# ShijieZhou-UCLA/feature-3dgs

Hardware: AMD Instinct MI355X
Metric: rendered Mpix/s of rasterizer fwd+bwd (train-step ms in ms_per_step), 1M Gaussians @1080p, feat_dim=32 (higher is better)
Workload: dtype f32 (blend-backward sums: bf16 x 2-term products, f32 accumulate); 1 GPU; c3: 1000000 Gaussians, 1920x1080, SH degree 3, feat_dim=32, one view per GPU (SURVEY.md 8d recipe, seed 0), fresh upstream gradients per step; P=1000000, parallelism=single GPU

## Files before the change

### feature-3dgs_amd/csrc/api.hip

```cpp

#include <algorithm>
#include <atomic>
#include <cstdarg>
#include <cstdio>
#include <cstdlib>
#include <cstring>
#include <initializer_list>
#include <limits>
#include <mutex>
#include <string>
#include <vector>

#include "common.h"

using namespace f3dgs;

namespace {

thread_local std::string g_err;
thread_local f3dgs_stage_fn g_feature_ready_fn = nullptr;
thread_local void* g_feature_ready_ctx = nullptr;
thread_local f3dgs_rows_fn g_rows_ready_fn = nullptr;
thread_local void* g_rows_ready_ctx = nullptr;
thread_local int g_rows_ready_chunks = 1;
// ... 95 lines not shown
    do {                                                                                       \
        hipError_t e_ = (expr);                                                                \
        if (e_ != hipSuccess) return fail(F3DGS_ERR_HIP, "%s failed: %s", #expr, hipGetErrorString(e_)); \
    } while (0)

bool profiling() { return options().profile != 0; }

struct PendingSpan {
    const char* name;
    hipEvent_t a, b;
};
std::mutex g_prof_mu;
std::vector<PendingSpan> g_pending;
std::vector<hipEvent_t> g_event_pool;
std::vector<std::pair<const char*, std::pair<double, long>>> g_totals;

void resolve_pending_locked();
constexpr size_t MAX_PENDING_SPANS = 4096;

hipEvent_t take_event_locked() {
    if (!g_event_pool.empty()) {
        hipEvent_t e = g_event_pool.back();
        g_event_pool.pop_back();
        return e;
    }
    hipEvent_t e = nullptr;
    (void)hipEventCreate(&e);
    return e;
}

struct StageTimer {
    hipStream_t s;
    bool on;
    bool blend_only;
    hipEvent_t prev;
    explicit StageTimer(hipStream_t st, bool allowed = true) : s(st), on(allowed && profiling()), blend_only(options().profile == 2), prev(nullptr) {
        if (on && !blend_only) {
            {
                std::lock_guard<std::mutex> lk(g_prof_mu);
                prev = take_event_locked();
            }
            (void)hipEventRecord(prev, s);
        }
    }
    ~StageTimer() {
        if (prev) {
            std::lock_guard<std::mutex> lk(g_prof_mu);
            g_pending.push_back({nullptr, prev, nullptr});
        }
    }
    StageTimer(const StageTimer&) = delete;
    StageTimer& operator=(const StageTimer&) = delete;
    void mark(const char* name) {
        if (!on) return;
        if (blend_only) {
            const bool opens = strcmp(name, "tile_sort") == 0 || strcmp(name, "zero") == 0;
            const bool closes = strcmp(name, "render_fwd") == 0 || strcmp(name, "render_bwd") == 0;
            if (!opens && !closes) return;
            hipEvent_t ev;
            {
                std::lock_guard<std::mutex> lk(g_prof_mu);
                if (g_pending.size() >= MAX_PENDING_SPANS) resolve_pending_locked();
                ev = take_event_locked();
            }
            (void)hipEventRecord(ev, s);
            if (opens) { prev = ev; return; }
            std::lock_guard<std::mutex> lk(g_prof_mu);
            if (prev) g_pending.push_back({name, prev, ev});
            g_pending.push_back({nullptr, ev, nullptr});
            prev = nullptr;
            return;
        }
        hipEvent_t e;
        {
            std::lock_guard<std::mutex> lk(g_prof_mu);
            if (g_pending.size() >= MAX_PENDING_SPANS) resolve_pending_locked();
            e = take_event_locked();
        }
        (void)hipEventRecord(e, s);
        {
            std::lock_guard<std::mutex> lk(g_prof_mu);
            g_pending.push_back({name, prev, e});
        }
        prev = e;
    }
};

void resolve_pending() {
    std::lock_guard<std::mutex> lk(g_prof_mu);
    resolve_pending_locked();
}

void resolve_pending_locked() {
    for (auto& p : g_pending) {
        if (p.name) {
            (void)hipEventSynchronize(p.b);
            float ms = 0;
            (void)hipEventElapsedTime(&ms, p.a, p.b);
            bool found = false;
            for (auto& t : g_totals)
                if (strcmp(t.first, p.name) == 0) { t.second.first += ms; t.second.second++; found = true; break; }
            if (!found) g_totals.push_back({p.name, {ms, 1}});
        } else {
            (void)hipEventSynchronize(p.a);
        }
        g_event_pool.push_back(p.a);
    }
    g_pending.clear();
}

int check_debug(int debug, hipStream_t s, const char* stage) {
    if (!debug) return F3DGS_OK;
    hipError_t e = hipStreamSynchronize(s);
    if (e == hipSuccess) e = hipGetLastError();
    if (e != hipSuccess) return fail(F3DGS_ERR_HIP, "stage '%s' failed: %s", stage, hipGetErrorString(e));
    return F3DGS_OK;
}

void fill_view(ViewParams& vp, const float* view, const float* proj, const float* campos, const float* bg, float tanx,
               float tany, int W, int H, float mod) {
    vp.view = view; vp.proj = proj; vp.campos = campos; vp.bg = bg;
    vp.tanx = tanx; vp.tany = tany;
    vp.fx = W / (2.0f * tanx); vp.fy = H / (2.0f * tany);
    vp.W = W; vp.H = H;
    vp.gx = (W + TILE - 1) / TILE; vp.gy = (H + TILE - 1) / TILE;
    vp.band0 = 0; vp.band1 = vp.gy;
    vp.scale_modifier = mod;
    vp.max_axis_ratio = 0.f;
}

int tile_cull_enabled() { return options().tile_cull ? 1 : 0; }

struct OptionDesc {
    const char* name;
    const char* env;
    int Options::*field;
    int dflt;
};
const OptionDesc kOptions[] = {
    {"tile_cull", "F3DGS_TILE_CULL", &Options::tile_cull, 1},
    {"feature_mfma", "F3DGS_FEATURE_MFMA", &Options::feature_mfma, 1},
    {"profile", "F3DGS_PROFILE", &Options::profile, 0},
    {"bwd_half", "F3DGS_BWD_HALF", &Options::bwd_half, 1},
    {"bwd_pl", "F3DGS_BWD_PL", &Options::bwd_pl, -1},
    {"bwd_order", "F3DGS_BWD_ORDER", &Options::bwd_order, 1},
    {"bwd_m44", "F3DGS_BWD_M44", &Options::bwd_m44, 1},
    {"bwd_split16", "F3DGS_BWD_SPLIT16", &Options::bwd_split16, 1},
    {"bwd_bf16", "F3DGS_BWD_BF16", &Options::bwd_bf16, -1},
    {"bwd_bf16_max_ratio", "F3DGS_BWD_BF16_MAX_RATIO", &Options::bwd_bf16_max_ratio, 16},
    {"bwd_wide8", "F3DGS_BWD_WIDE8", &Options::bwd_wide8, 1},
    {"fwd_wide", "F3DGS_FWD_WIDE", &Options::fwd_wide, 1},
    {"fwd_solo", "F3DGS_FWD_SOLO", &Options::fwd_solo, 1},
    {"sort_onesweep", "F3DGS_SORT_ONESWEEP", &Options::sort_onesweep, 0},
    {"sync_free", "F3DGS_SYNC_FREE", &Options::sync_free, -1},
    {"instance_capacity", "F3DGS_INSTANCE_CAPACITY", &Options::instance_capacity, 0},
    {"knn_outward", "F3DGS_KNN_OUTWARD", &Options::knn_outward, 1},
#ifdef F3DGS_DEV
    {"dev", "F3DGS_DEV_BITS", &Options::dev, 0},
#endif
};

bool misaligned16(std::initializer_list<const void*> ptrs) {
    uintptr_t bits = 0;
    for (const void* p : ptrs) bits |= reinterpret_cast<uintptr_t>(p);
    return (bits & 15) != 0;
}

int tile_bits(int tiles) {
    int b = 0;
    while ((1 << b) < tiles) b++;
    return b < 1 ? 1 : b;
}

}

namespace f3dgs {
Options& options() {
    static Options o = [] {
        Options v{};
        for (const OptionDesc& d : kOptions) {
            const char* e = getenv(d.env);
            v.*(d.field) = e ? atoi(e) : d.dflt;
        }
        return v;
    }();
    return o;
}
}

namespace {
struct CountReadback {
    uint32_t* host = nullptr;
    uint32_t* dev = nullptr;
    hipEvent_t done = nullptr;
    int device = -1;
    hipStream_t stream = nullptr;
    bool in_graph = false;
};
struct CountHint { bool known = false; uint32_t own = 0, ref = 0; };
thread_local CountHint g_count_hint[64];
thread_local const uint32_t* g_last_forward_words = nullptr;
bool stream_is_capturing(hipStream_t s) {
    hipStreamCaptureStatus st = hipStreamCaptureStatusNone;
    if (hipStreamIsCapturing(s, &st) != hipSuccess) { (void)hipGetLastError(); return false; }
    return st == hipStreamCaptureStatusActive;
}
const hipStream_t kSpareSlot = reinterpret_cast<hipStream_t>(~uintptr_t(0));
bool make_count_slot(std::vector<CountReadback>& slots, int dev, hipStream_t s) {
    CountReadback rb;
    void* p = nullptr;
    if (hipHostMalloc(&p, 64, hipHostMallocPortable | hipHostMallocMapped) != hipSuccess) { (void)hipGetLastError(); return false; }
    rb.host = static_cast<uint32_t*>(p);
    void* d = nullptr;
    if (hipHostGetDevicePointer(&d, p, 0) != hipSuccess || hipEventCreateWithFlags(&rb.done, hipEventDisableTiming) != hipSuccess) {
        (void)hipGetLastError();
        (void)hipHostFree(p);
        return false;
    }
    rb.dev = static_cast<uint32_t*>(d);
    rb.device = dev;
    rb.stream = s;
    memset(p, 0, 64);
    if (slots.size() >= 64) {
        for (size_t i = 0; i < slots.size(); i++)
            if (!slots[i].in_graph && slots[i].stream != kSpareSlot) {
                (void)hipEventDestroy(slots[i].done);
                (void)hipHostFree(slots[i].host);
                slots.erase(slots.begin() + (long)i);
                break;
            }
    }
    slots.push_back(rb);
    return true;
}
CountReadback* count_readback(hipStream_t s, bool may_create) {
    thread_local std::vector<CountReadback> slots;
    int dev = 0;
    if (hipGetDevice(&dev) != hipSuccess) return nullptr;
    auto find = [&](hipStream_t key) -> CountReadback* {
        for (CountReadback& rb : slots)
            if (rb.device == dev && rb.stream == key) return &rb;
        return nullptr;
    };
    if (!may_create) {
        if (CountReadback* rb = find(s)) return rb;
        if (CountReadback* spare = find(kSpareSlot)) { spare->stream = s; return spare; }
        return nullptr;
    }
    if (!find(kSpareSlot)) (void)make_count_slot(slots, dev, kSpareSlot);
    if (!find(s) && !make_count_slot(slots, dev, s)) return nullptr;
    return find(s);
}
}

extern "C" {

int f3dgs_version(void) { return 32200; }

int f3dgs_last_backward_contraction(void) { return g_last_bwd_bf16.load(); }

const uint32_t* f3dgs_forward_counts(void) { return g_last_forward_words; }

int f3dgs_set_option(const char* name, int value) {
    if (!name) return fail(F3DGS_ERR_INVALID_ARGUMENT, "null option name");
    for (const OptionDesc& d : kOptions)
        if (strcmp(d.name, name) == 0) {
            options().*(d.field) = value;
            return F3DGS_OK;
        }
    return fail(F3DGS_ERR_INVALID_ARGUMENT, "unknown option '%s'", name);
}

int f3dgs_get_option(const char* name, int* value) {
    if (!name || !value) return fail(F3DGS_ERR_INVALID_ARGUMENT, "null argument");
    for (const OptionDesc& d : kOptions)
        if (strcmp(d.name, name) == 0) {
            *value = options().*(d.field);
            return F3DGS_OK;
        }
    return fail(F3DGS_ERR_INVALID_ARGUMENT, "unknown option '%s'", name);
}

const char* f3dgs_option_name(int index) {
    const int n = (int)(sizeof(kOptions) / sizeof(kOptions[0]));
    return (index >= 0 && index < n) ? kOptions[index].name : nullptr;
}

const char* f3dgs_last_error(void) { return g_err.c_str(); }

void f3dgs_set_feature_grad_ready_callback(f3dgs_stage_fn fn, void* ctx) {
    g_feature_ready_fn = fn;
    g_feature_ready_ctx = ctx;
}

void f3dgs_set_feature_grad_accumulate(int on) { g_feature_accumulate = on ? 1 : 0; }

int f3dgs_set_feature_grad_lowres(const float* gx, int Hg, int Wg, const float* scale) {
    if (!gx) { g_lowres = LowresGrad(); return F3DGS_OK; }
    if (Hg <= 0 || Wg <= 0) return fail(F3DGS_ERR_INVALID_ARGUMENT, "bad low-resolution size %d x %d", Hg, Wg);
    g_lowres.gx = gx; g_lowres.scale = scale; g_lowres.Hg = Hg; g_lowres.Wg = Wg;
    return F3DGS_OK;
}

int f3dgs_debug_band_order(int gx, int gy, int tile_row_begin, int tile_row_end, uint32_t* tiles_out) {
    if (gx <= 0 || gy <= 0 || !tiles_out) return fail(F3DGS_ERR_INVALID_ARGUMENT, "bad grid");
    int b0r, b1r;
    clamp_band(tile_row_begin, tile_row_end, gy, &b0r, &b1r);
    uint32_t b0 = 0, tb = 0;
    band_perm_params(gx, gy, b0r, b1r, &b0, &tb);
    const uint32_t T = (uint32_t)gx * (uint32_t)gy;
    for (uint32_t v = 0; v < T; v++) tiles_out[v] = band_perm(v, T, b0, tb);
    return tb != 0 ? 1 : 0;
}

void f3dgs_set_tile_band(int tile_row_begin, int tile_row_end) {
    g_band_begin = tile_row_begin;
    g_band_end = tile_row_end;
}

void f3dgs_set_grad_rows_ready_callback(f3dgs_rows_fn fn, void* ctx, int chunks) {
    g_rows_ready_fn = fn;
    g_rows_ready_ctx = ctx;
    g_rows_ready_chunks = chunks > 0 ? chunks : 1;
}

int f3dgs_mark_visible(int P, const float* means3D, const float* viewmatrix, const float* projmatrix,
                       uint8_t* present, void* stream) {
    hipStream_t s = static_cast<hipStream_t>(stream);
    if (P < 0) return fail(F3DGS_ERR_INVALID_ARGUMENT, "P < 0");
    if (P == 0) return F3DGS_OK;
    if (!means3D || !viewmatrix || !present) return fail(F3DGS_ERR_INVALID_ARGUMENT, "null pointer");
    (void)projmatrix;
    launch_mark_visible(P, means3D, viewmatrix, present, s);
    HIP_TRY(hipGetLastError());
    return F3DGS_OK;
}

int f3dgs_forward(f3dgs_resize_fn geometry_resize, void* geometry_ctx, f3dgs_resize_fn binning_resize,
                  void* binning_ctx, f3dgs_resize_fn image_resize, void* image_ctx, int P, int D, int M, int C,
                  const float* background, int width, int height, const float* means3D, const float* shs,
                  const float* colors_precomp, const float* semantic_feature, const float* opacities,
                  const float* scales, float scale_modifier, const float* rotations, const float* cov3D_precomp,
                  const float* viewmatrix, const float* projmatrix, const float* cam_pos, float tan_fovx,
                  float tan_fovy, int prefiltered, float* out_color, float* out_feature_map, float* out_depth,
                  int* radii, int debug, void* stream, int* num_rendered) {
    hipStream_t s = static_cast<hipStream_t>(stream);
    (void)prefiltered;
    if (num_rendered) *num_rendered = 0;
    if (P < 0 || C < 0 || width <= 0 || height <= 0) return fail(F3DGS_ERR_INVALID_ARGUMENT, "bad sizes");
    if (!geometry_resize || !binning_resize || !image_resize) return fail(F3DGS_ERR_INVALID_ARGUMENT, "null resize hook");
    if (!out_color || !out_depth || (C > 0 && !out_feature_map)) return fail(F3DGS_ERR_INVALID_ARGUMENT, "null output");
    const size_t HW = (size_t)width * height;
    if (P == 0) {
        const bool cap0 = stream_is_capturing(s);
        HIP_TRY(zero_fill(out_color, 3 * HW * sizeof(float), cap0, s));
        HIP_TRY(zero_fill(out_depth, HW * sizeof(float), cap0, s));
        if (C) HIP_TRY(zero_fill(out_feature_map, (size_t)C * HW * sizeof(float), cap0, s));
        return F3DGS_OK;
    }
    if (!means3D || !opacities || !viewmatrix || !projmatrix || !background)
        return fail(F3DGS_ERR_INVALID_ARGUMENT, "null input");
    if (!colors_precomp && !shs) return fail(F3DGS_ERR_INVALID_ARGUMENT, "need shs or colors_precomp");
    if (!colors_precomp && !cam_pos) return fail(F3DGS_ERR_INVALID_ARGUMENT, "SH colours need cam_pos");
    if (!cov3D_precomp && (!scales || !rotations))
        return fail(F3DGS_ERR_INVALID_ARGUMENT, "need scales+rotations or cov3D_precomp");
    if (C > 0 && !semantic_feature) return fail(F3DGS_ERR_INVALID_ARGUMENT, "semantic_feature is null but C > 0");
    if (shs && (D < 0 || D > 3 || (D + 1) * (D + 1) > M))
        return fail(F3DGS_ERR_INVALID_ARGUMENT, "SH degree %d needs %d coefficients, M = %d", D, (D + 1) * (D + 1), M);
    if (misaligned16({shs, rotations, semantic_feature}))
        return fail(F3DGS_ERR_INVALID_ARGUMENT, "shs, rotations and semantic_feature must be 16-byte aligned (f3dgs.h, Alignment)");

    int rc = F3DGS_OK;
    ViewParams vp;
    fill_view(vp, viewmatrix, projmatrix, cam_pos, background, tan_fovx, tan_fovy, width, height, scale_modifier);
    vp.max_axis_ratio = 1.001f * (float)options().bwd_bf16_max_ratio;
    if (g_band_begin != 0 || g_band_end != 0) clamp_band(g_band_begin, g_band_end, vp.gy, &vp.band0, &vp.band1);
    const int2 band = make_int2(vp.band0, vp.band1);
    const size_t tiles = (size_t)vp.gx * vp.gy;

    size_t geom_bytes = 0, img_bytes = 0, bin_bytes = 0;
    GeomState::carve(nullptr, P, &geom_bytes);
    char* geom_ptr = geometry_resize(geometry_ctx, geom_bytes);
    if (!geom_ptr) return fail(F3DGS_ERR_ALLOC, "geometry buffer allocation of %zu bytes failed", geom_bytes);
    GeomState geom = GeomState::carve(geom_ptr, P, nullptr);
    ImageState::carve(nullptr, HW, tiles, &img_bytes);
    char* img_ptr = image_resize(image_ctx, img_bytes);
    if (!img_ptr) return fail(F3DGS_ERR_ALLOC, "image buffer allocation of %zu bytes failed", img_bytes);
    ImageState img = ImageState::carve(img_ptr, HW, tiles, nullptr);
    const bool onesweep = options().sort_onesweep != 0 && tiles <= 65536;

    const bool capturing = stream_is_capturing(s);
    const int sf_opt = options().sync_free;
    const bool sync_free = !onesweep && (sf_opt > 0 || (sf_opt < 0 && capturing));
    if (capturing && !sync_free)
        return fail(F3DGS_ERR_UNSUPPORTED, "the stream is being captured into a graph: the forward call reads the instance count on the host "
                    "unless option sync_free is 1 or -1 (and sort_onesweep = 0)");
    if (capturing && debug) return fail(F3DGS_ERR_UNSUPPORTED, "debug = 1 synchronises after every stage: not inside a graph capture");
    int dev_index = 0;
    HIP_TRY(hipGetDevice(&dev_index));
    if (dev_index < 0 || dev_index >= 64) return fail(F3DGS_ERR_UNSUPPORTED, "device index %d", dev_index);
    CountHint& hint = g_count_hint[dev_index];

    StageTimer tm(s, !capturing);
    const int cull = tile_cull_enabled();
    launch_preprocess(P, D, M, means3D, scales, rotations, opacities, shs, cov3D_precomp, colors_precomp, vp, radii,
                      geom, cull, s);
    if ((rc = check_debug(debug, s, "preprocess"))) return rc;
    tm.mark("preprocess");
    if (onesweep) launch_sort_prologue(geom, (size_t)P, s);
    CountReadback* rbp = count_readback(s, !capturing);
    if (!rbp)
        return capturing ? fail(F3DGS_ERR_UNSUPPORTED, "graph capture: run one forward call on this stream (same host thread) before capturing - "
                                "the pinned count words are allocated on a stream's first call")
                         : fail(F3DGS_ERR_ALLOC, "pinned read-back buffer / event creation failed");
    CountReadback& rb = *rbp;
    if (capturing) rb.in_graph = true;
    g_last_forward_words = rb.host;
    if (onesweep) {
        HIP_TRY(hipMemcpyAsync(rb.host, geom.counters, 8, hipMemcpyDeviceToHost, s));
        HIP_TRY(hipEventRecord(rb.done, s));
    }

    const TotalsJob tj = {geom.ref_partial, (P + 255) / 256, geom.counters, rb.dev, capturing ? nullptr : rb.done};
    const OffsetSumsJob sums = {geom.tiles_touched, geom.scan_tmp, geom.scan_sub};
    bool sums_done = false;
    bool counts_in_a = false;
    if (onesweep) launch_depth_sort_onesweep(geom, (size_t)P, s);
    else HIP_TRY(launch_depth_sort(geom.depth_key, geom.key_a, geom.val_a, geom.key_b, geom.val_b, (size_t)P, geom.hist, &tj, s, &sums, &sums_done, &counts_in_a));
    if ((rc = check_debug(debug, s, "depth sort"))) return rc;
    tm.mark("depth_sort");
    const uint32_t* order = geom.val_a;
    const uint32_t* counts_in_order = counts_in_a ? geom.key_a : nullptr;

    if (!onesweep && !sums_done) {
        if (counts_in_order) launch_offset_sums(counts_in_order, nullptr, (size_t)P, geom.scan_tmp, geom.scan_sub, s);
        else launch_offset_sums(geom.tiles_touched, order, (size_t)P, geom.scan_tmp, geom.scan_sub, s);
    }

    bool known = false;
    uint32_t N = 0, n_ref = 0, cap = 0;
    auto read_counts = [&]() -> int {
        HIP_TRY(hipEventSynchronize(rb.done));
        N = rb.host[0]; n_ref = rb.host[1];
        note_frame(geom_ptr, (onesweep || rb.host[2] != 0u) ? 1.f : 0.f, vp.band0, vp.band1);
        hint.known = true; hint.own = N; hint.ref = n_ref;
        known = true;
        if (N >= (1u << 30) || n_ref >= (1u << 31)) return fail(F3DGS_ERR_UNSUPPORTED, "more than 2^30 instances");
        return F3DGS_OK;
    };
    if (sync_free && (options().instance_capacity > 0 || hint.known)) {
        unsigned long long want = options().instance_capacity > 0 ? (unsigned long long)options().instance_capacity
                                                                  : (unsigned long long)hint.own + hint.own / 4 + 4096ull;
        if (options().instance_capacity <= 0 && hint.own <= (uint32_t)SMALL_SORT_MAX && want > (unsigned long long)SMALL_SORT_MAX)
            want = SMALL_SORT_MAX;
        cap = (uint32_t)std::min(want, (1ull << 30) - 1ull);
    } else if (capturing) {
        return fail(F3DGS_ERR_UNSUPPORTED, "graph capture: no provision for the instance lists - run one forward call on this thread and device "
                    "before capturing, or set option instance_capacity");
    } else {
        if ((rc = read_counts())) return rc;
        cap = N;
    }
    tm.mark("scan+sync");

    const int bits = tile_bits((int)tiles);
    const int passes = (bits + RADIX_BITS - 1) / RADIX_BITS;
    BinState bin;
    for (;;) {
        const uint32_t n_carve = known ? N : cap;
        BinState::carve(nullptr, n_carve, &bin_bytes, tiles);
        char* bin_ptr = binning_resize(binning_ctx, bin_bytes);
        if (!bin_ptr) return fail(F3DGS_ERR_ALLOC, "binning buffer allocation of %zu bytes failed", bin_bytes);
        bin = BinState::carve(bin_ptr, n_carve, nullptr, tiles);
        rb.host[3] = n_carve;
        uint32_t* in_tile = (passes % 2 == 0) ? bin.tile_sorted : bin.tile_tmp;
        uint32_t* in_id = (passes % 2 == 0) ? bin.point_list : bin.id_tmp;
        if (onesweep) {
            HIP_TRY(hipMemsetAsync(img.tile_len, 0, tiles * sizeof(uint32_t), s));
            launch_emit_scan(P, geom, bin, order, vp.gx, vp.gy, band, cull, in_tile, in_id, N, bin.ranges_enc, s);
            if ((rc = check_debug(debug, s, "emit"))) return rc;
            tm.mark("emit");
            launch_tile_sort_onesweep(geom, bin, N, passes, bin.ranges_enc, s);
            if ((rc = check_debug(debug, s, "tile sort"))) return rc;
            tm.mark("tile_sort");
        } else if (known && N == 0) {
            HIP_TRY(hipMemsetAsync(bin.ranges_enc, 0xFF, tiles * sizeof(uint2), s));
            HIP_TRY(hipMemsetAsync(img.tile_len, 0, tiles * sizeof(uint32_t), s));
        } else {
            launch_emit_instances(P, geom, order, counts_in_order, vp.gx, vp.gy, band, cull, in_tile, in_id, bin.ranges_enc, img.tile_len, n_carve,
                                  known ? nullptr : geom.counters, capturing ? rb.dev + 4 : nullptr, s);
            if ((rc = check_debug(debug, s, "emit"))) return rc;
            tm.mark("emit");
            launch_radix_sort_pairs(bin.tile_sorted, bin.point_list, bin.tile_tmp, bin.id_tmp, n_carve, bits, bin.hist, true,
                                    bin.ranges_enc, s, known ? nullptr : geom.counters);
            if ((rc = check_debug(debug, s, "tile sort"))) return rc;
            tm.mark("tile_sort");
        }

        launch_render_forward(vp, C, bin.ranges_enc, img.ranges, bin.point_list, geom.rec, semantic_feature, img.final_T,
                              img.n_contrib, out_color, out_feature_map, out_depth, img.tile_len, s);
        if ((rc = check_debug(debug, s, "render"))) return rc;
        tm.mark("render_fwd");
        if (known || capturing) break;
        if ((rc = read_counts())) return rc;
        if (N <= cap) break;
    }
    if (capturing) {
        note_frame(geom_ptr, 2.f, vp.band0, vp.band1);
        n_ref = std::max(1u, hint.ref);
    }
    if (num_rendered) *num_rendered = (int)n_ref;
    HIP_TRY(hipGetLastError());
    return F3DGS_OK;
}

size_t f3dgs_backward_scratch_bytes(int P, int C) {
    (void)C;
    return ((size_t)(P > 0 ? P : 0) * GREC * sizeof(float) + ALIGN - 1) & ~(ALIGN - 1);
}

int f3dgs_backward(int P, int D, int M, int C, int R, const float* background, int width, int height,
                   const float* means3D, const float* shs, const float* colors_precomp,
                   const float* semantic_feature, const float* scales, float scale_modifier, const float* rotations,
                   const float* cov3D_precomp, const float* viewmatrix, const float* projmatrix, const float* campos,
                   float tan_fovx, float tan_fovy, const int* radii, const char* geom_buffer,
                   const char* binning_buffer, const char* image_buffer, const float* dL_dpix,
                   const float* dL_dfeaturepix, const float* dL_depths, float* dL_dmean2D, float* dL_dconic,
                   float* dL_dopacity, float* dL_dcolor, float* dL_dsemantic_feature, float* dL_dmean3D,
                   float* dL_dcov3D, float* dL_dsh, float* dL_dscale, float* dL_drot, float* dL_dz, void* scratch,
                   int debug, void* stream) {
    hipStream_t s = static_cast<hipStream_t>(stream);
    (void)semantic_feature;
    (void)colors_precomp;
    const LowresGrad lowres = g_lowres;
    g_lowres = LowresGrad();
    if (P < 0 || C < 0 || R < 0) return fail(F3DGS_ERR_INVALID_ARGUMENT, "bad sizes");
    if (P == 0) return F3DGS_OK;
    if (!geom_buffer || !image_buffer || (R > 0 && !binning_buffer))
        return fail(F3DGS_ERR_INVALID_ARGUMENT, "null state buffer");
    if (!radii) return fail(F3DGS_ERR_INVALID_ARGUMENT, "radii is required");
    if (lowres.gx) {
        if (C == 0) return fail(F3DGS_ERR_INVALID_ARGUMENT, "a low-resolution feature-map gradient was set but C = 0");
        if (lowres.Hg > height || lowres.Wg > width)
            return fail(F3DGS_ERR_UNSUPPORTED, "low-resolution feature-map gradient %d x %d is larger than the image %d x %d: "
                        "apply the transposed resize outside (f3dgs_feature_l1 with d_feature_map)", lowres.Hg, lowres.Wg, height, width);
        if (!options().feature_mfma)
            return fail(F3DGS_ERR_UNSUPPORTED, "the low-resolution feature-map gradient is taken by the pixel-lane backward (option feature_mfma = 1)");
    }
    if (!dL_dpix || !dL_depths || (C > 0 && !dL_dfeaturepix && !lowres.gx)) return fail(F3DGS_ERR_INVALID_ARGUMENT, "null upstream grad");
    if (!dL_dmean2D || !dL_dopacity || !dL_dcolor || !dL_dmean3D || !dL_dcov3D || (C > 0 && !dL_dsemantic_feature))
        return fail(F3DGS_ERR_INVALID_ARGUMENT, "null output");
    if (M > 0 && shs && !dL_dsh) return fail(F3DGS_ERR_INVALID_ARGUMENT, "dL_dsh is null");
    if (shs && dL_dsh && (D < 0 || D > 3 || (D + 1) * (D + 1) > M))
        return fail(F3DGS_ERR_INVALID_ARGUMENT, "SH degree %d needs %d coefficients, M = %d", D, (D + 1) * (D + 1), M);
    if (scales && (!dL_dscale || !dL_drot || !rotations)) return fail(F3DGS_ERR_INVALID_ARGUMENT, "scale/rot grads null");
    if (!scratch) return fail(F3DGS_ERR_INVALID_ARGUMENT, "scratch is null");
    if (misaligned16({shs, rotations, dL_dsh, dL_drot, dL_dconic, dL_dsemantic_feature, scratch}))
        return fail(F3DGS_ERR_INVALID_ARGUMENT, "shs, rotations, dL_dsh, dL_drot, dL_dconic, dL_dsemantic_feature and scratch must be "
                    "16-byte aligned (f3dgs.h, Alignment)");

    int rc = F3DGS_OK;
    ViewParams vp;
    fill_view(vp, viewmatrix, projmatrix, campos, background, tan_fovx, tan_fovy, width, height, scale_modifier);
    const size_t HW = (size_t)width * height, tiles = (size_t)vp.gx * vp.gy;
    GeomState geom = GeomState::carve(const_cast<char*>(geom_buffer), P, nullptr);
    const uint32_t* point_list = BinState::list_of(binning_buffer);
    ImageState img = ImageState::carve(const_cast<char*>(image_buffer), HW, tiles, nullptr);
    float* grec = static_cast<float*>(scratch);

    const bool capturing = stream_is_capturing(s);
    if (capturing && debug) return fail(F3DGS_ERR_UNSUPPORTED, "debug = 1 synchronises after every stage: not inside a graph capture");
    StageTimer tm(s, !capturing);
    HIP_TRY(zero_fill(grec, (size_t)P * GREC * sizeof(float), capturing, s));
    if (C > 0 && !g_feature_accumulate) HIP_TRY(zero_fill(dL_dsemantic_feature, (size_t)P * C * sizeof(float), capturing, s));
    tm.mark("zero");
    int contraction = options().bwd_bf16 > 0 ? 1 : 0;
    {
        float long_axis = 1.f;
        const bool noted = frame_note(geom_buffer, vp.gy, &long_axis, &vp.band0, &vp.band1);
        if (options().bwd_bf16 < 0) {
            contraction = (noted && long_axis == 0.f) ? 1 : 2;
// ... 461 lines not shown
```

### feature-3dgs_amd/csrc/binding.cpp

```cpp

#include <ATen/hip/impl/HIPGuardImplMasqueradingAsCUDA.h>
#include <ATen/hip/impl/HIPStreamMasqueradingAsCUDA.h>
#include <torch/extension.h>

#include <array>
#include <exception>
#include <stdexcept>
#include <string>
#include <tuple>
#include <vector>

#include "../../include/f3dgs.h"

namespace py = pybind11;

namespace {

const float* fptr(const torch::Tensor& t) { return t.numel() ? t.data_ptr<float>() : nullptr; }

char* resize_hook(void* ctx, size_t n) {
    auto* t = static_cast<torch::Tensor*>(ctx);
    t->resize_({(long long)n});
    return reinterpret_cast<char*>(t->data_ptr());
}
// ... 1072 lines not shown
                "densify_gather: override_row must be int32 of the same length");
    TORCH_CHECK(srcs.size() == dsts.size() && srcs.size() == modes.size() && srcs.size() == overrides.size(), "densify_gather: list lengths differ");
    std::vector<f3dgs_densify_tensor> table(srcs.size());
    for (size_t i = 0; i < srcs.size(); i++) {
        const auto& a = srcs[i];
        auto& d = dsts[i];
        TORCH_CHECK(a.is_cuda() && d.is_cuda() && a.scalar_type() == torch::kFloat32 && d.scalar_type() == torch::kFloat32, "densify_gather: float32 HIP tensors only");
        TORCH_CHECK(a.is_contiguous() && d.is_contiguous(), "densify_gather: contiguous tensors only");
        int64_t width = 1;
        for (int64_t k = 1; k < a.dim(); k++) width *= a.size(k);
        TORCH_CHECK(a.dim() >= 1 && width >= 1, "densify_gather: tensors are (rows, ...) with non-empty rows");
        TORCH_CHECK((size_t)d.numel() >= n_out * (size_t)width, "densify_gather: destination ", i, " too small");
        table[i].src = a.data_ptr<float>();
        table[i].dst = d.data_ptr<float>();
        table[i].width = (int)width;
        table[i].mode = (int)modes[i];
        table[i].override_src = nullptr;
        if (modes[i] == F3DGS_DENSIFY_OVERRIDE_CHILD) {
            const auto& o = overrides[i];
            TORCH_CHECK(o.is_cuda() && o.scalar_type() == torch::kFloat32 && o.is_contiguous(), "densify_gather: override must be a contiguous float32 HIP tensor");
            table[i].override_src = o.numel() ? o.data_ptr<float>() : a.data_ptr<float>();
        }
    }
    c10::hip::HIPGuardMasqueradingAsCUDA guard(src_row.device());
    check_status(f3dgs_densify_gather(n_out, src_row.data_ptr<int32_t>(), kind.data_ptr<uint8_t>(), override_row.data_ptr<int32_t>(),
                                      (int)table.size(), table.data(), current_stream(src_row)),
                 "densify_gather");
}

}

PYBIND11_MODULE(_C, m) {
    m.def("rasterize_gaussians", &RasterizeGaussians);
    m.def("rasterize_gaussians_backward", &RasterizeGaussiansBackward);
    m.def("mark_visible", &markVisible);
    m.def("feature_l1", &FeatureL1, py::arg("feature_map"), py::arg("gt"), py::arg("weight"), py::arg("bias"), py::arg("dense") = true);
    m.def("set_feature_grad_lowres", [](py::object gx, py::object scale) {
              auto& h = feature_grad_lowres();
              h.first = gx.is_none() ? torch::Tensor() : gx.cast<torch::Tensor>();
              h.second = (gx.is_none() || scale.is_none()) ? torch::Tensor() : scale.cast<torch::Tensor>();
          },
          py::arg("gx"), py::arg("scale") = py::none(),
          "gx (Hg, Wg, C) float32 = dL/d(resized feature map) as feature_l1 returns it, scale = 0-dim device tensor or None: the NEXT "
          "rasterize_gaussians_backward call takes its feature-map gradient from there (transposed resize applied per tile); None clears");
    m.def("feature_decode", &FeatureDecode);
    m.def("image_loss_forward", &ImageLossForward, py::arg("image"), py::arg("gt"), py::arg("lambda_dssim"), py::arg("want_grad"),
          py::arg("per_image") = false);
    m.def("image_loss_backward", &ImageLossBackward, py::arg("image"), py::arg("gt"), py::arg("scratch"), py::arg("upstream"),
          py::arg("lambda_dssim"), py::arg("mode"));
    m.attr("IMAGE_LOSS_L1_DSSIM") = (int)F3DGS_IMAGE_LOSS_L1_DSSIM;
    m.attr("IMAGE_LOSS_SSIM") = (int)F3DGS_IMAGE_LOSS_SSIM;
    m.attr("IMAGE_LOSS_SSIM_PER_IMAGE") = (int)F3DGS_IMAGE_LOSS_SSIM_PER_IMAGE;
    m.def("image_metrics", &ImageMetrics, py::arg("image"), py::arg("gt"), py::arg("image_format"), py::arg("gt_format"), py::arg("flags"),
          py::arg("want_ssim") = true);
    m.attr("IMAGE_F32") = (int)F3DGS_IMAGE_F32;
    m.attr("IMAGE_U8_PLANAR") = (int)F3DGS_IMAGE_U8_PLANAR;
    m.attr("IMAGE_U8_INTERLEAVED") = (int)F3DGS_IMAGE_U8_INTERLEAVED;
    m.attr("METRICS_QUANTIZE_IMAGE") = (int)F3DGS_METRICS_QUANTIZE_IMAGE;
    m.attr("METRICS_QUANTIZE_GT") = (int)F3DGS_METRICS_QUANTIZE_GT;
    m.def("edit_select", &EditSelect, py::arg("features"), py::arg("text"), py::arg("positive_mask"), py::arg("first_positive"),
          py::arg("variant"), py::arg("threshold") = py::none(), py::arg("normalize_inplace") = false, py::arg("want_score") = false,
          py::arg("opacity") = py::none());
    m.def("segment", &Segment, py::arg("feature_map"), py::arg("text"), py::arg("Hs"), py::arg("Ws"), py::arg("weight"), py::arg("bias"),
          py::arg("flags"), py::arg("want_score"));
    m.def("contributions", &Contributions, py::arg("geomBuffer"), py::arg("binningBuffer"), py::arg("imgBuffer"), py::arg("P"),
          py::arg("num_rendered"), py::arg("H"), py::arg("W"), py::arg("masks") = py::none(), py::arg("acc") = py::none(),
          py::arg("wmax") = py::none(), py::arg("want_pixel") = true);
    m.attr("CONTRIB_MAX_MASKS") = (int)F3DGS_CONTRIB_MAX_MASKS;
    m.def("label_votes", &LabelVotes, py::arg("geomBuffer"), py::arg("binningBuffer"), py::arg("imgBuffer"), py::arg("P"),
          py::arg("num_rendered"), py::arg("H"), py::arg("W"), py::arg("labels"), py::arg("L"), py::arg("acc"));
    m.attr("LABEL_VOTES_MAX_LABELS") = (int)F3DGS_LABEL_VOTES_MAX_LABELS;
    m.def("instance_associate", &InstanceAssociate, py::arg("acc_view"), py::arg("acc"), py::arg("count"), py::arg("dropped"),
          py::arg("iou_thresh"), py::arg("min_weight"));
    m.def("instance_merge", &InstanceMerge, py::arg("acc_view"), py::arg("mapping"), py::arg("acc"), py::arg("clear_view"));
    m.attr("INSTANCE_MAX_MASKS") = (int)F3DGS_INSTANCE_MAX_MASKS;
    m.attr("INSTANCE_MAX_INSTANCES") = (int)F3DGS_INSTANCE_MAX_INSTANCES;
    m.def("feature_pca_moments", &FeaturePcaMoments, py::arg("feature_map"), py::arg("stride"));
    m.def("feature_pca_project", &FeaturePcaProject, py::arg("feature_map"), py::arg("mean"), py::arg("components"),
          py::arg("lo") = py::none(), py::arg("hi") = py::none());
    m.attr("FEATURE_PCA_MAX_CHANNELS") = (int)F3DGS_FEATURE_PCA_MAX_CHANNELS;
    m.def("view_normals", &ViewNormals, py::arg("depth"), py::arg("projection_matrix"), py::arg("inv_full_proj"), py::arg("chw") = false,
          py::arg("half") = false);
    m.def("view_gradient", &ViewGradient, py::arg("image"));
    m.def("view_curvature", &ViewCurvature, py::arg("depth"), py::arg("projection_matrix"), py::arg("inv_full_proj"));
    m.def("view_minmax", &ViewMinmax, py::arg("field"));
    m.def("view_palette", &ViewPalette, py::arg("field"), py::arg("minmax"), py::arg("lut"), py::arg("mode"), py::arg("want_float") = true,
          py::arg("want_u8") = false);
    m.def("view_bytes", &ViewBytes, py::arg("image"));
    m.attr("VIEW_TILE") = (int)F3DGS_VIEW_TILE;
    m.attr("VIEW_PALETTE_MINMAX") = (int)F3DGS_VIEW_PALETTE_MINMAX;
    m.attr("VIEW_PALETTE_MAX") = (int)F3DGS_VIEW_PALETTE_MAX;
    m.attr("VIEW_PALETTE_MAX_ENTRIES") = (int)F3DGS_VIEW_PALETTE_MAX_ENTRIES;
    m.attr("SEGMENT_ROUND_HALF") = (int)F3DGS_SEGMENT_ROUND_HALF;
    m.attr("SEGMENT_TEXT_NORMALIZED") = (int)F3DGS_SEGMENT_TEXT_NORMALIZED;
    m.attr("SEGMENT_MAX_TEXTS") = (int)F3DGS_SEGMENT_MAX_TEXTS;
    m.def("seg_metrics", &SegMetrics, py::arg("teacher"), py::arg("student"), py::arg("gt"), py::arg("num_labels"), py::arg("num_classes"),
          py::arg("carry_counts"), py::arg("carry_scalars"), py::arg("want_scores"));
    m.def("seg_colorize", &SegColorize, py::arg("labels"), py::arg("palette"), py::arg("image"), py::arg("mode"), py::arg("a"), py::arg("b"),
          py::arg("fill"));
    m.def("sam_masks", &SamMasks, py::arg("low_res"), py::arg("iou_preds"), py::arg("pred_iou_thresh"), py::arg("S"), py::arg("ih"),
          py::arg("iw"), py::arg("H"), py::arg("W"), py::arg("FH"), py::arg("FW"), py::arg("cx0"), py::arg("cy0"), py::arg("t"), py::arg("t_hi"),
          py::arg("t_lo"), py::arg("stability_thresh"), py::arg("edge_filter"));
    m.def("sam_upscale", &SamUpscale, py::arg("low_res"), py::arg("S"), py::arg("ih"), py::arg("iw"), py::arg("H"), py::arg("W"), py::arg("t"),
          py::arg("out_bool"));
    m.def("box_nms", &BoxNms, py::arg("boxes"), py::arg("categories"), py::arg("iou_threshold"), py::arg("order"));
    m.def("mask_rle_count", &MaskRleCount, py::arg("packed"), py::arg("index"), py::arg("FH"));
    m.def("mask_rle_emit", &MaskRleEmit, py::arg("packed"), py::arg("index"), py::arg("FH"), py::arg("lens"), py::arg("ends"), py::arg("out"),
          py::arg("head"));
    m.def("mask_unpack", &MaskUnpack, py::arg("packed"), py::arg("index"), py::arg("FH"));
    m.def("mask_instance_map", &MaskInstanceMap, py::arg("packed"), py::arg("index"), py::arg("FH"));
    m.def("mask_regions", &MaskRegions, py::arg("packed"), py::arg("index"), py::arg("FH"), py::arg("area_thresh"), py::arg("holes"),
          py::arg("run_capacity"));
    m.attr("BOX_NMS_MAX") = (int)F3DGS_BOX_NMS_MAX;
    m.attr("LABELS_U8") = (int)F3DGS_LABELS_U8;
    m.attr("LABELS_I32") = (int)F3DGS_LABELS_I32;
    m.attr("LABELS_I64") = (int)F3DGS_LABELS_I64;
    m.attr("SEG_COLOR_MASK") = (int)F3DGS_SEG_COLOR_MASK;
    m.attr("SEG_COLOR_BLEND") = (int)F3DGS_SEG_COLOR_BLEND;
    m.attr("SEG_COLOR_STRIP") = (int)F3DGS_SEG_COLOR_STRIP;
    m.attr("EDIT_SELECT") = (int)F3DGS_EDIT_SELECT;
    m.attr("EDIT_DELETE") = (int)F3DGS_EDIT_DELETE;
    m.attr("EDIT_TEXT_NORMALIZED") = (int)F3DGS_EDIT_TEXT_NORMALIZED;
    m.attr("EDIT_FILL_UNSELECTED") = (int)F3DGS_EDIT_FILL_UNSELECTED;
    m.attr("EDIT_MAX_TEXTS") = (int)F3DGS_EDIT_MAX_TEXTS;
    m.attr("EDIT_MAX_TEXT_ELEMENTS") = (int)F3DGS_EDIT_MAX_TEXT_ELEMENTS;
    m.def("adam_step", &AdamStep, py::arg("param"), py::arg("grad"), py::arg("exp_avg"), py::arg("exp_avg_sq"), py::arg("lr"),
          py::arg("beta1"), py::arg("beta2"), py::arg("eps"), py::arg("step"), py::arg("row_mask") = py::none());
    m.def("adam_step_multi", &AdamStepMulti, py::arg("params"), py::arg("grads"), py::arg("exp_avgs"), py::arg("exp_avg_sqs"), py::arg("lrs"),
          py::arg("beta1"), py::arg("beta2"), py::arg("eps"), py::arg("steps"), py::arg("row_mask") = py::none());
    m.def("densify_gather", &DensifyGather);
    m.def("version", []() { return f3dgs_version(); });
    m.def("set_feature_grad_hook", [](py::object fn) { feature_grad_hook() = std::move(fn); },
          "callable(dL_dsemantic_feature) run inside rasterize_gaussians_backward once that tensor is final on the stream; None removes it");
    m.def("set_feature_grad_accumulator", [](py::object t) {
              if (t.is_none()) feature_grad_accumulator() = torch::Tensor();
              else feature_grad_accumulator() = t.cast<torch::Tensor>();
          },
          "tensor (P*C float32, contiguous, on the op's device) that the following backward calls ADD dL/dsemantic_feature into "
          "(they then return an empty tensor for that gradient); None restores the default");
    m.def("set_grad_rows_hook", [](py::object fn, int chunks) { grad_rows_hook() = std::move(fn); grad_rows_chunks() = chunks > 0 ? chunks : 1; },
          py::arg("fn"), py::arg("chunks") = 4,
          "callable(row_begin, row_end, grads: dict) run inside rasterize_gaussians_backward after each of `chunks` row ranges of the "
          "per-Gaussian gradients is final on the stream; None removes it");
    m.def("set_option", [](const std::string& name, int value) { check_status(f3dgs_set_option(name.c_str(), value), "set_option"); });
    m.def("set_tile_band", [](int row_begin, int row_end) { f3dgs_set_tile_band(row_begin, row_end); }, py::arg("tile_row_begin"), py::arg("tile_row_end"),
          "forward calls of this thread list and blend only tile rows [begin, end) of the view (0, 0: the whole view); include/f3dgs.h");
    m.def("forward_counts", []() -> py::object {
        const uint32_t* w = f3dgs_forward_counts();
        if (!w) return py::none();
        const volatile uint32_t* v = w;
        return py::make_tuple((long long)v[0], (long long)v[1], (long long)v[2], (long long)v[3], (long long)v[4]);
    }, "(entries of the instance lists, the reference's num_rendered, long-axis flag, entries provided for, sticky no-room word) of the "
       "calling thread's most recent forward call - final once that frame's work has completed; None before the first call");
    m.def("forward_counts_address", []() { return (uintptr_t)f3dgs_forward_counts(); },
          "host address of the five uint32 words of forward_counts() (0 before the first call): a captured step keeps it and reads the words after a replay");
    m.def("clear_forward_overflow", [](uintptr_t address) { if (address) reinterpret_cast<volatile uint32_t*>(address)[4] = 0u; },
          "clears the sticky no-room word behind an address returned by forward_counts_address()");
    m.def("last_backward_contraction", []() { return f3dgs_last_backward_contraction(); },
          "1: the last blend backward of this process contracted on bf16 matrix instructions (two-term operands); 0: exact fp32; -1: none yet");
    m.def("get_option", [](const std::string& name) {
        int v = 0;
        check_status(f3dgs_get_option(name.c_str(), &v), "get_option");
        return v;
    });
    m.def("profile_reset", []() { f3dgs_profile_reset(); });
    m.def("profile_read", []() {
        const char* names[64];
        double ms[64];
        long calls[64];
        const int n = f3dgs_profile_read(names, ms, calls, 64);
        std::vector<std::tuple<std::string, double, long>> out;
        for (int i = 0; i < n; i++) out.emplace_back(names[i], ms[i], calls[i]);
        return out;
    });
}
```

### feature-3dgs_amd/csrc/binning.hip

```cpp

#include <atomic>
#include "common.h"
#include "lookback.h"

namespace f3dgs {

namespace {

__global__ void __launch_bounds__(256) scan_reduce_kernel(const uint32_t* __restrict__ in,
                                                          const uint32_t* __restrict__ gather, size_t n,
                                                          uint32_t* __restrict__ block_sums, uint32_t* __restrict__ sub) {
    __shared__ uint32_t sh[8];
    const size_t base = (size_t)blockIdx.x * SCAN_CHUNK;
    const int lane = threadIdx.x & 63, w = threadIdx.x >> 6;
    uint32_t v[16];
#pragma unroll
    for (int k = 0; k < 16; k++) {
        const size_t i = base + (size_t)k * 256 + threadIdx.x;
        v[k] = i < n ? (gather ? in[gather[i]] : in[i]) : 0u;
    }
    uint32_t acc = 0;
#pragma unroll
    for (int k = 0; k < 16; k++) {
        uint32_t r = v[k];
#pragma unroll
        for (int d = 32; d >= 1; d >>= 1) r += (uint32_t)__shfl_xor((int)r, d, 64);
        if (lane == 0) sub[(size_t)blockIdx.x * 64 + 4 * k + w] = r;
        acc += v[k];
    }
    uint32_t tot;
    block_excl_scan_256(acc, sh, &tot);
    if (threadIdx.x == 0) block_sums[blockIdx.x] = tot;
}


template <int THREADS>
__device__ __forceinline__ void run_totals_job(const TotalsJob& tj) {
    __shared__ uint32_t shc[3][THREADS / 64];
    uint32_t v = 0, u = 0, ar = 0;
    for (int i = threadIdx.x; i < tj.n_partial; i += THREADS) {
        v += tj.partial[i]; u += tj.partial[tj.n_partial + i]; ar = max(ar, tj.partial[2 * tj.n_partial + i]);
    }
#pragma unroll
    for (int d = 32; d >= 1; d >>= 1) {
        v += (uint32_t)__shfl_xor((int)v, d, 64);
        u += (uint32_t)__shfl_xor((int)u, d, 64);
        ar = max(ar, (uint32_t)__shfl_xor((int)ar, d, 64));
    }
    if ((threadIdx.x & 63) == 0) { shc[0][threadIdx.x >> 6] = v; shc[1][threadIdx.x >> 6] = u; shc[2][threadIdx.x >> 6] = ar; }
    __syncthreads();
    if (threadIdx.x == 0) {
        uint32_t ref = 0, own = 0, arm = 0;
        for (int k = 0; k < THREADS / 64; k++) { ref += shc[0][k]; own += shc[1][k]; arm = max(arm, shc[2][k]); }
        tj.counters[0] = own; tj.counters[1] = ref; tj.counters[2] = arm; tj.counters[3] = 0u;
        if (tj.host) {
            __hip_atomic_store(&tj.host[0], own, __ATOMIC_RELAXED, __HIP_MEMORY_SCOPE_SYSTEM);
            __hip_atomic_store(&tj.host[1], ref, __ATOMIC_RELAXED, __HIP_MEMORY_SCOPE_SYSTEM);
            __hip_atomic_store(&tj.host[2], arm, __ATOMIC_RELAXED, __HIP_MEMORY_SCOPE_SYSTEM);
            __threadfence_system();
        }
    }
}

template <int BITS, int ITEMS>
__global__ void __launch_bounds__(SORT_THREADS) radix_hist_kernel(const uint32_t* __restrict__ keys, size_t n,
                                                                  int shift, uint32_t nb,
                                                                  uint32_t* __restrict__ hist, TotalsJob tj,
                                                                  const uint32_t* __restrict__ n_dev) {
    constexpr int BINS = 1 << BITS;
    constexpr int CHUNK = SORT_THREADS * ITEMS;
    __shared__ uint32_t h[BINS];
    if (n_dev) { const size_t nd = *n_dev; n = nd <= n ? nd : 0; }
    const size_t base = (size_t)blockIdx.x * CHUNK;
    uint32_t key[ITEMS];
#pragma unroll
    for (int k = 0; k < ITEMS; k++) {
        const size_t i = base + (size_t)k * SORT_THREADS + threadIdx.x;
        key[k] = i < n ? keys[i] : 0u;
    }
    if (tj.partial && blockIdx.x == 0) run_totals_job<SORT_THREADS>(tj);
    for (int d = threadIdx.x; d < BINS; d += SORT_THREADS) h[d] = 0;
    __syncthreads();
#pragma unroll
    for (int k = 0; k < ITEMS; k++) {
        const size_t i = base + (size_t)k * SORT_THREADS + threadIdx.x;
        if (i < n) atomicAdd(&h[(key[k] >> shift) & (BINS - 1)], 1u);
    }
    __syncthreads();
    for (int d = threadIdx.x; d < BINS; d += SORT_THREADS) hist[(size_t)d * nb + blockIdx.x] = h[d];
}

constexpr int ROWSCAN_GROUPS = 8;
__global__ void __launch_bounds__(256) radix_rowscan_kernel(uint32_t* __restrict__ hist, uint32_t nb,
                                                            uint32_t* __restrict__ totals) {
    __shared__ uint32_t sh[8];
    __shared__ uint4 wtot[ROWSCAN_GROUPS];
    uint32_t* row = hist + (size_t)blockIdx.x * nb;
    const int lane = threadIdx.x & 63, w = threadIdx.x >> 6;
    uint32_t v[ROWSCAN_GROUPS], inc[ROWSCAN_GROUPS];
#pragma unroll
    for (int k = 0; k < ROWSCAN_GROUPS; k++) {
        const uint32_t i = (uint32_t)k * 256 + threadIdx.x;
        const uint32_t r = row[i < nb ? i : 0u];
        v[k] = i < nb ? r : 0u;
    }
#pragma unroll
    for (int k = 0; k < ROWSCAN_GROUPS; k++) {
        inc[k] = (uint32_t)k * 256 < nb ? wave_incl_scan(v[k], lane) : 0u;
        if (lane == 63) (&wtot[k].x)[w] = inc[k];
    }
    __syncthreads();
    uint32_t carry = 0;
#pragma unroll
    for (int k = 0; k < ROWSCAN_GROUPS; k++) {
        const uint4 t = wtot[k];
        const uint32_t before = carry + (w > 0 ? t.x : 0u) + (w > 1 ? t.y : 0u) + (w > 2 ? t.z : 0u);
        const uint32_t i = (uint32_t)k * 256 + threadIdx.x;
        if (i < nb) row[i] = before + inc[k] - v[k];
        carry += t.x + t.y + t.z + t.w;
    }
    for (uint32_t base = ROWSCAN_GROUPS * 256; base < nb; base += 256) {
        const uint32_t i = base + threadIdx.x;
        const uint32_t v = i < nb ? row[i] : 0;
        uint32_t tot;
        const uint32_t ex = block_excl_scan_256(v, sh, &tot);
        if (i < nb) row[i] = carry + ex;
        carry += tot;
    }
    if (threadIdx.x == 0) totals[blockIdx.x] = carry;
}

__device__ __forceinline__ void record_range(uint2* ranges_enc, uint32_t tile, bool first, bool last, uint32_t pos) {
    if (first) atomicMin(&ranges_enc[tile].x, pos);
    if (last) atomicMin(&ranges_enc[tile].y, 0xFFFFFFFFu - (pos + 1u));
}

template <int BITS, int ITEMS, bool REORDER, bool RANGES, bool COUNTS = false>
__global__ void __launch_bounds__(SORT_THREADS)
radix_scatter_kernel(const uint32_t* __restrict__ keys_in, const uint32_t* __restrict__ vals_in,
                     uint32_t* __restrict__ keys_out, uint32_t* __restrict__ vals_out, size_t n, int shift,
                     uint32_t nb, const uint32_t* __restrict__ hist, const uint32_t* __restrict__ totals,
                     uint2* __restrict__ ranges_enc, const uint32_t* __restrict__ n_dev,
                     const uint32_t* __restrict__ payload) {
    constexpr int BINS = 1 << BITS;
    constexpr int CHUNK = SORT_THREADS * ITEMS;
    constexpr int BPT = BINS >= SORT_THREADS ? BINS / SORT_THREADS : 1;
    static_assert(BINS >= SORT_THREADS ? BINS % SORT_THREADS == 0 : true, "whole bins per thread");
    if (n_dev) {
        const size_t nd = *n_dev;
        n = nd <= n ? nd : 0;
        if ((size_t)blockIdx.x * CHUNK >= n) return;
    }
    __shared__ uint32_t cnt[4][BINS];
    __shared__ uint32_t sh[8];
    __shared__ uint32_t gbase[REORDER ? BINS : 1];
    __shared__ uint32_t lstart[REORDER ? BINS : 1];
    __shared__ uint32_t skey[REORDER ? CHUNK : 1];
    __shared__ uint32_t sval[REORDER ? CHUNK : 1];
    volatile uint32_t* vcnt = &cnt[0][0];
    const int lane = threadIdx.x & 63, w = threadIdx.x >> 6;
    for (int d = threadIdx.x; d < 4 * BINS; d += SORT_THREADS) (&cnt[0][0])[d] = 0;
    __syncthreads();

    const size_t wbase = (size_t)blockIdx.x * CHUNK + (size_t)w * (ITEMS * 64);
    uint32_t key[ITEMS];
    constexpr bool VAL_FIRST = REORDER || COUNTS;
    uint32_t val[VAL_FIRST ? ITEMS : 1];
    uint32_t rank[ITEMS];
    const unsigned long long lt_mask = (1ull << lane) - 1ull;
#pragma unroll
    for (int k = 0; k < ITEMS; k++) {
        const size_t i = wbase + (size_t)k * 64 + lane;
        key[k] = i < n ? keys_in[i] : 0xFFFFFFFFu;
        if constexpr (VAL_FIRST) val[k] = (vals_in && i < n) ? vals_in[i] : (uint32_t)i;
    }
#pragma unroll
    for (int k = 0; k < ITEMS; k++) {
        const size_t i = wbase + (size_t)k * 64 + lane;
        const bool valid = i < n;
        const uint32_t d = (key[k] >> shift) & (BINS - 1);
        const unsigned long long vm = __ballot(valid);
        uint32_t p_lo = (uint32_t)vm, p_hi = (uint32_t)(vm >> 32);
#pragma unroll
        for (int b = 0; b < BITS; b++) {
            const uint32_t x = 0u - ((d >> b) & 1u);
            const unsigned long long nm = ~__ballot(x != 0u);
            p_lo &= (uint32_t)nm ^ x;
            p_hi &= (uint32_t)(nm >> 32) ^ x;
        }
        const unsigned long long peers = ((unsigned long long)p_hi << 32) | p_lo;
        const uint32_t before = __popcll(peers & lt_mask);
        const uint32_t old = vcnt[w * BINS + d];
        if (valid && before == 0) vcnt[w * BINS + d] = old + (uint32_t)__popcll(peers);
        rank[k] = old + before;
    }
    uint32_t pay[(COUNTS && !REORDER) ? ITEMS : 1];
    (void)pay;
    if constexpr (COUNTS && !REORDER) {
#pragma unroll
        for (int k = 0; k < ITEMS; k++) {
            const size_t i = wbase + (size_t)k * 64 + lane;
            pay[k] = payload[i < n ? val[k] : 0u];
        }
    }
    __syncthreads();
    {
        uint32_t tot[BPT], run = 0, blk[BPT], brun = 0;
#pragma unroll
        for (int q = 0; q < BPT; q++) {
            const uint32_t d = threadIdx.x * BPT + q;
            const bool own = BINS >= SORT_THREADS || d < (uint32_t)BINS;
            tot[q] = own ? totals[d] : 0u;
            run += tot[q];
            blk[q] = own ? cnt[0][d] + cnt[1][d] + cnt[2][d] + cnt[3][d] : 0u;
            brun += blk[q];
        }
        uint32_t digit_base = block_excl_scan_256(run, sh, nullptr);
        uint32_t local_base = REORDER ? block_excl_scan_256(brun, sh, nullptr) : 0;
#pragma unroll
        for (int q = 0; q < BPT; q++) {
            const uint32_t d = threadIdx.x * BPT + q;
            if (BINS < SORT_THREADS && d >= (uint32_t)BINS) break;
            const uint32_t g = digit_base + hist[(size_t)d * nb + blockIdx.x];
            if (REORDER) { gbase[d] = g; lstart[d] = local_base; }
            uint32_t r2 = REORDER ? local_base : g;
#pragma unroll
            for (int k = 0; k < 4; k++) {
                const uint32_t c = cnt[k][d];
                cnt[k][d] = r2;
                r2 += c;
            }
            digit_base += tot[q];
            local_base += blk[q];
        }
    }
    __syncthreads();
    if (REORDER) {
#pragma unroll
        for (int k = 0; k < ITEMS; k++) {
            const size_t i = wbase + (size_t)k * 64 + lane;
            if (i < n) {
                const uint32_t d = (key[k] >> shift) & (BINS - 1);
                const uint32_t lp = cnt[w][d] + rank[k];
                skey[lp] = key[k];
                if constexpr (REORDER) sval[lp] = val[k];
            }
        }
        __syncthreads();
        const size_t cbase = (size_t)blockIdx.x * CHUNK;
        const uint32_t have = (uint32_t)min((size_t)CHUNK, n - cbase);
        if constexpr (COUNTS) {
            static_assert(!RANGES, "the depth sort records no ranges");
            uint32_t pos[ITEMS], id[ITEMS], c[ITEMS];
#pragma unroll
            for (int k = 0; k < ITEMS; k++) {
                const uint32_t j = (uint32_t)k * SORT_THREADS + threadIdx.x;
                const uint32_t jj = j < have ? j : 0u;
                const uint32_t d = (skey[jj] >> shift) & (BINS - 1);
                pos[k] = gbase[d] + (jj - lstart[d]);
                id[k] = sval[jj];
                c[k] = payload[id[k]];
            }
#pragma unroll
            for (int k = 0; k < ITEMS; k++) {
                const uint32_t j = (uint32_t)k * SORT_THREADS + threadIdx.x;
                if (j < have) {
                    keys_out[pos[k]] = c[k];
                    vals_out[pos[k]] = id[k];
                }
            }
        } else {
#pragma unroll
            for (int k = 0; k < ITEMS; k++) {
                const uint32_t j = (uint32_t)k * SORT_THREADS + threadIdx.x;
                if (j < have) {
                    const uint32_t kk = skey[j];
                    const uint32_t d = (kk >> shift) & (BINS - 1);
                    const uint32_t pos = gbase[d] + (j - lstart[d]);
                    keys_out[pos] = kk;
                    vals_out[pos] = sval[j];
                    if (RANGES) record_range(ranges_enc, kk, j == 0 || skey[j - 1] != kk, j + 1 == have || skey[j + 1] != kk, pos);
                }
            }
        }
    } else {
#pragma unroll
        for (int k = 0; k < ITEMS; k++) {
            const size_t i = wbase + (size_t)k * 64 + lane;
            if (i < n) {
                const uint32_t d = (key[k] >> shift) & (BINS - 1);
                const uint32_t pos = cnt[w][d] + rank[k];
                if constexpr (COUNTS) {
                    keys_out[pos] = pay[k];
                    vals_out[pos] = val[k];
                } else {
                    keys_out[pos] = key[k];
                    vals_out[pos] = vals_in ? vals_in[i] : (uint32_t)i;
                }
            }
        }
    }
}


template <int ITEMS, bool WRITE_KEYS, bool RANGES>
__global__ void __launch_bounds__(SORT_THREADS)
onesweep_pass_kernel(const uint32_t* __restrict__ keys_in, const uint32_t* __restrict__ vals_in,
                     uint32_t* __restrict__ keys_out, uint32_t* __restrict__ vals_out, size_t n, int shift,
                     const uint32_t* __restrict__ digit_totals, uint32_t* __restrict__ status,
                     uint32_t* __restrict__ ticket, uint2* __restrict__ ranges) {
    constexpr int BINS = 256;
    constexpr int CHUNK = SORT_THREADS * ITEMS;
    __shared__ uint32_t cnt[4][BINS];
    __shared__ uint32_t sh[8];
    __shared__ uint32_t gbase[BINS];
    __shared__ uint32_t lstart[BINS];
    __shared__ uint32_t skey[CHUNK];
    __shared__ uint32_t sval[CHUNK];
    __shared__ uint32_t s_vb;
    volatile uint32_t* vcnt = &cnt[0][0];
    const int lane = threadIdx.x & 63, w = threadIdx.x >> 6;
    if (threadIdx.x == 0) s_vb = atomicAdd(ticket, 1u);
    for (int d = threadIdx.x; d < 4 * BINS; d += SORT_THREADS) (&cnt[0][0])[d] = 0;
    __syncthreads();
    const uint32_t vb = s_vb;

    const size_t cbase = (size_t)vb * CHUNK;
    const size_t wbase = cbase + (size_t)w * (ITEMS * 64);
    uint32_t key[ITEMS];
    uint32_t rank[ITEMS];
    const unsigned long long lt_mask = (1ull << lane) - 1ull;
#pragma unroll
    for (int k = 0; k < ITEMS; k++) {
        const size_t i = wbase + (size_t)k * 64 + lane;
        const bool valid = i < n;
        key[k] = valid ? keys_in[i] : 0xFFFFFFFFu;
        const uint32_t d = (key[k] >> shift) & (BINS - 1);
        unsigned long long peers = __ballot(valid);
#pragma unroll
        for (int b = 0; b < 8; b++) {
            const bool bit = (d >> b) & 1;
            const unsigned long long m = __ballot(bit);
            peers &= bit ? m : ~m;
        }
        const uint32_t before = __popcll(peers & lt_mask);
        const uint32_t old = vcnt[w * BINS + d];
        if (valid && before == 0) vcnt[w * BINS + d] = old + (uint32_t)__popcll(peers);
        rank[k] = old + before;
    }
    __syncthreads();
    {
        const uint32_t d = threadIdx.x;
        const uint32_t blk = cnt[0][d] + cnt[1][d] + cnt[2][d] + cnt[3][d];
        const uint32_t total = digit_totals[d];
        const uint32_t digit_base = block_excl_scan_256(total, sh, nullptr);
        const uint32_t local_base = block_excl_scan_256(blk, sh, nullptr);
        const uint32_t before_me = lookback(status + d, BINS, vb, blk);
        gbase[d] = digit_base + before_me;
        lstart[d] = local_base;
        uint32_t r2 = local_base;
#pragma unroll
        for (int k = 0; k < 4; k++) {
            const uint32_t c = cnt[k][d];
            cnt[k][d] = r2;
            r2 += c;
        }
    }
    __syncthreads();
#pragma unroll
    for (int k = 0; k < ITEMS; k++) {
        const size_t i = wbase + (size_t)k * 64 + lane;
        if (i < n) {
            const uint32_t d = (key[k] >> shift) & (BINS - 1);
            const uint32_t lp = cnt[w][d] + rank[k];
            skey[lp] = key[k];
            sval[lp] = vals_in ? vals_in[i] : (uint32_t)i;
        }
    }
    __syncthreads();
    const uint32_t have = (uint32_t)min((size_t)CHUNK, n - cbase);
#pragma unroll
    for (int k = 0; k < ITEMS; k++) {
        const uint32_t j = (uint32_t)k * SORT_THREADS + threadIdx.x;
        if (j < have) {
            const uint32_t kk = skey[j];
            const uint32_t d = (kk >> shift) & (BINS - 1);
            const uint32_t pos = gbase[d] + (j - lstart[d]);
            if (WRITE_KEYS) keys_out[pos] = kk;
            vals_out[pos] = sval[j];
            if (RANGES) record_range(ranges, kk, j == 0 || skey[j - 1] != kk, j + 1 == have || skey[j + 1] != kk, pos);
        }
    }
}

__global__ void __launch_bounds__(256)
sort_prologue_kernel(const uint32_t* __restrict__ keys, size_t n, uint32_t* __restrict__ depth_hist,
                     const uint32_t* __restrict__ partial, int n_partial, uint32_t* __restrict__ counters,
                     uint32_t* __restrict__ zero_words, size_t n_zero) {
    __shared__ uint32_t h[4][256];
    __shared__ uint32_t shc[2][4];
    for (int d = threadIdx.x; d < 1024; d += 256) (&h[0][0])[d] = 0;
    for (size_t i = (size_t)blockIdx.x * 256 + threadIdx.x; i < n_zero; i += (size_t)gridDim.x * 256) zero_words[i] = 0;
    __syncthreads();
    const size_t base = (size_t)blockIdx.x * SCAN_CHUNK;
    uint32_t culled = 0;
#pragma unroll
    for (int k = 0; k < 16; k++) {
        const size_t i = base + (size_t)k * 256 + threadIdx.x;
        if (i < n) {
            const uint32_t kk = keys[i];
            if (kk == 0xFFFFFFFFu) { culled++; continue; }
            atomicAdd(&h[0][kk & 255], 1u);
            atomicAdd(&h[1][(kk >> 8) & 255], 1u);
            atomicAdd(&h[2][(kk >> 16) & 255], 1u);
            atomicAdd(&h[3][kk >> 24], 1u);
        }
    }
#pragma unroll
    for (int d = 32; d >= 1; d >>= 1) culled += (uint32_t)__shfl_xor((int)culled, d, 64);
    if ((threadIdx.x & 63) == 0 && culled)
        for (int p = 0; p < 4; p++) atomicAdd(&h[p][255], culled);
    __syncthreads();
    for (int p = 0; p < 4; p++) {
        const uint32_t c = h[p][threadIdx.x];
        if (c) atomicAdd(&depth_hist[p * 256 + threadIdx.x], c);
    }
    if (blockIdx.x == 0) {
        uint32_t v = 0, u = 0;
        for (int i = threadIdx.x; i < n_partial; i += 256) { v += partial[i]; u += partial[n_partial + i]; }
#pragma unroll
        for (int d = 32; d >= 1; d >>= 1) {
            v += (uint32_t)__shfl_xor((int)v, d, 64);
            u += (uint32_t)__shfl_xor((int)u, d, 64);
        }
        if ((threadIdx.x & 63) == 0) { shc[0][threadIdx.x >> 6] = v; shc[1][threadIdx.x >> 6] = u; }
        __syncthreads();
        if (threadIdx.x == 0) {
            counters[1] = shc[0][0] + shc[0][1] + shc[0][2] + shc[0][3];
            counters[0] = shc[1][0] + shc[1][1] + shc[1][2] + shc[1][3];
            counters[3] = 0u;
        }
    }
}
// ... 15 lines not shown
constexpr int SMALL_SORT_THREADS = 1024;
constexpr int SMALL_SORT_ITEMS = SMALL_SORT_MAX / SMALL_SORT_THREADS;
struct SmallSortLds {
    uint32_t key[SMALL_SORT_MAX];
    uint32_t val[SMALL_SORT_MAX];
    uint32_t cnt[SMALL_SORT_THREADS / 64][256];
    uint32_t wsum[4];
};
template <bool RANGES>
__global__ void __launch_bounds__(SMALL_SORT_THREADS)
small_sort_kernel(const uint32_t* __restrict__ keys_in, const uint32_t* __restrict__ vals_in, uint32_t* __restrict__ keys_out,
                  uint32_t* __restrict__ vals_out, uint32_t n, int passes, TotalsJob tj, uint2* __restrict__ ranges_enc,
                  const uint32_t* __restrict__ n_dev, OffsetSumsJob os) {
    extern __shared__ __attribute__((aligned(16))) char small_sort_smem[];
    SmallSortLds& L = *reinterpret_cast<SmallSortLds*>(small_sort_smem);
    constexpr int ITEMS = SMALL_SORT_ITEMS, NW = SMALL_SORT_THREADS / 64;
    if (n_dev) { const uint32_t nd = *n_dev; n = nd <= n ? nd : 0u; }
    if (tj.partial) run_totals_job<SMALL_SORT_THREADS>(tj);
    const int tid = threadIdx.x, lane = tid & 63, w = tid >> 6;
    const unsigned long long lt_mask = (1ull << lane) - 1ull;
    volatile uint32_t* vcnt = &L.cnt[w][0];
    const int steps = (int)((n + SMALL_SORT_THREADS - 1) / SMALL_SORT_THREADS);
    const uint32_t wbase = (uint32_t)(w * steps * 64 + lane);
    uint32_t key[ITEMS], val[ITEMS], rank[ITEMS];
#pragma unroll
    for (int k = 0; k < ITEMS; k++) {
        const uint32_t i = wbase + (uint32_t)(k * 64);
        const bool mine = k < steps && i < n;
        key[k] = mine ? keys_in[i] : 0xFFFFFFFFu;
        val[k] = (vals_in && mine) ? vals_in[i] : i;
    }
    for (int pass = 0; pass < passes; pass++) {
        const int shift = 8 * pass;
        for (int d = tid; d < NW * 256; d += SMALL_SORT_THREADS) (&L.cnt[0][0])[d] = 0;
        __syncthreads();
#pragma unroll
        for (int k = 0; k < ITEMS; k++) {
            if (k >= steps) break;
            const uint32_t i = wbase + (uint32_t)(k * 64);
            const bool valid = i < n;
            const uint32_t d = (key[k] >> shift) & 255u;
            const unsigned long long vm = __ballot(valid);
            uint32_t p_lo = (uint32_t)vm, p_hi = (uint32_t)(vm >> 32);
#pragma unroll
            for (int b = 0; b < 8; b++) {
                const uint32_t x = 0u - ((d >> b) & 1u);
                const unsigned long long nm = ~__ballot(x != 0u);
                p_lo &= (uint32_t)nm ^ x;
                p_hi &= (uint32_t)(nm >> 32) ^ x;
            }
            const unsigned long long peers = ((unsigned long long)p_hi << 32) | p_lo;
            const uint32_t before = __popcll(peers & lt_mask);
            const uint32_t old = vcnt[d];
            if (valid && before == 0) vcnt[d] = old + (uint32_t)__popcll(peers);
            rank[k] = old + before;
        }
        __syncthreads();
        {
            uint32_t tot = 0;
            if (tid < 256) {
#pragma unroll
                for (int ww = 0; ww < NW; ww++) tot += L.cnt[ww][tid];
            }
            uint32_t inc = tot;
#pragma unroll
            for (int d = 1; d < 64; d <<= 1) {
                const uint32_t v = (uint32_t)__shfl_up((int)inc, d, 64);
                if (lane >= d) inc += v;
            }
            if (tid < 256 && lane == 63) L.wsum[w] = inc;
            __syncthreads();
            if (tid < 256) {
                uint32_t base = inc - tot;
                for (int ww = 0; ww < w; ww++) base += L.wsum[ww];
#pragma unroll
                for (int ww = 0; ww < NW; ww++) {
                    const uint32_t c = L.cnt[ww][tid];
                    L.cnt[ww][tid] = base;
                    base += c;
                }
            }
        }
        __syncthreads();
#pragma unroll
        for (int k = 0; k < ITEMS; k++) {
            const uint32_t i = wbase + (uint32_t)(k * 64);
            if (k < steps && i < n) {
                const uint32_t pos = L.cnt[w][(key[k] >> shift) & 255u] + rank[k];
                L.key[pos] = key[k];
                L.val[pos] = val[k];
            }
        }
        __syncthreads();
        if (pass + 1 < passes) {
#pragma unroll
            for (int k = 0; k < ITEMS; k++) {
                const uint32_t i = wbase + (uint32_t)(k * 64);
                if (k < steps && i < n) { key[k] = L.key[i]; val[k] = L.val[i]; }
            }
        }
    }
#pragma unroll
    for (int k = 0; k < ITEMS; k++) {
        const uint32_t j = (uint32_t)(k * SMALL_SORT_THREADS + tid);
        if (j < n) {
            const uint32_t kk = L.key[j];
            if (keys_out) keys_out[j] = kk;
            vals_out[j] = L.val[j];
            if (RANGES) record_range(ranges_enc, kk, j == 0 || L.key[j - 1] != kk, j + 1 == n || L.key[j + 1] != kk, j);
        }
    }
    if (os.tiles_touched) {
        static_assert(SCAN_CHUNK == 64 * 64 && SMALL_SORT_THREADS == 1024, "run = item / 64, chunk = run / 64");
        const uint32_t nchunks = (n + SCAN_CHUNK - 1) / SCAN_CHUNK;
        uint32_t* const runs = &L.cnt[0][0];
#pragma unroll
        for (int k = 0; k < ITEMS; k++) {
            const uint32_t j = (uint32_t)(k * SMALL_SORT_THREADS + tid);
            uint32_t r = j < n ? os.tiles_touched[L.val[j]] : 0u;
#pragma unroll
            for (int d = 32; d >= 1; d >>= 1) r += (uint32_t)__shfl_xor((int)r, d, 64);
            const uint32_t run = (uint32_t)(16 * k + w);
            if (lane == 0) {
                runs[run] = r;
                if (run < 64u * nchunks) os.sub[run] = r;
            }
        }
        __syncthreads();
        if ((uint32_t)tid < nchunks) {
            uint32_t t = 0;
            for (int q = 0; q < 64; q++) t += runs[64 * tid + q];
            os.chunk_sums[tid] = t;
        }
    }
}

__global__ void __launch_bounds__(256) totals_kernel(TotalsJob tj) { run_totals_job<256>(tj); }

template <bool RANGES>
bool small_sort_usable() {
    constexpr int MAX_DEV = 64;
    static std::atomic<int> state[MAX_DEV];
    int dev = 0;
    if (hipGetDevice(&dev) != hipSuccess || dev < 0 || dev >= MAX_DEV) return false;
    if (state[dev].load(std::memory_order_acquire) == 0) {
        const hipError_t e = hipFuncSetAttribute(reinterpret_cast<const void*>(&small_sort_kernel<RANGES>),
                                                 hipFuncAttributeMaxDynamicSharedMemorySize, (int)sizeof(SmallSortLds));
        if (e != hipSuccess) (void)hipGetLastError();
        state[dev].store(e == hipSuccess ? 1 : -1, std::memory_order_release);
    }
    return state[dev].load(std::memory_order_acquire) > 0;
}

template <int BITS, int ITEMS>
static hipError_t radix_pass(const uint32_t* ki, const uint32_t* vi, uint32_t* ko, uint32_t* vo, size_t n, int shift,
                             uint32_t* hist, hipStream_t s, uint2* ranges_enc = nullptr, const TotalsJob* tj = nullptr,
                             const uint32_t* n_dev = nullptr, const uint32_t* payload = nullptr) {
    hipError_t rc = hipSuccess;
    constexpr int BINS = 1 << BITS;
    static_assert(ITEMS >= SORT_ITEMS, "the histogram buffers are sized for SORT_ITEMS keys per thread");
    const uint32_t nb = (uint32_t)((n + SORT_THREADS * ITEMS - 1) / (SORT_THREADS * ITEMS));
    uint32_t* totals = hist + (size_t)BINS * nb;
    hipLaunchKernelGGL((radix_hist_kernel<BITS, ITEMS>), dim3(nb), dim3(SORT_THREADS), 0, s, ki, n, shift, nb, hist,
                       tj ? *tj : TotalsJob{nullptr, 0, nullptr, nullptr}, n_dev);
    if (tj && tj->ready) rc = hipEventRecord(tj->ready, s);
    hipLaunchKernelGGL(radix_rowscan_kernel, dim3(BINS), dim3(256), 0, s, hist, nb, totals);
    const uint32_t* const no_payload = nullptr;
    if constexpr (ITEMS == SORT_ITEMS && (BITS == RADIX_BITS || BITS == DEPTH_RADIX_BITS)) {
        if (payload) {
            hipLaunchKernelGGL((radix_scatter_kernel<BITS, ITEMS, (BITS <= 8), false, true>), dim3(nb), dim3(SORT_THREADS), 0, s, ki,
                               vi, ko, vo, n, shift, nb, hist, totals, (uint2*)nullptr, n_dev, payload);
            return rc;
        }
    }
    if (ranges_enc && BITS <= 8)
        hipLaunchKernelGGL((radix_scatter_kernel<BITS, ITEMS, true, true>), dim3(nb), dim3(SORT_THREADS), 0, s, ki, vi, ko, vo, n,
                           shift, nb, hist, totals, ranges_enc, n_dev, no_payload);
    else
        hipLaunchKernelGGL((radix_scatter_kernel<BITS, ITEMS, (BITS <= 8), false>), dim3(nb), dim3(SORT_THREADS), 0, s, ki, vi, ko,
                           vo, n, shift, nb, hist, totals, (uint2*)nullptr, n_dev, no_payload);
    return rc;
}

static void tile_radix_pass(int bits, const uint32_t* ki, const uint32_t* vi, uint32_t* ko, uint32_t* vo, size_t n, int shift,
                            uint32_t* hist, hipStream_t s, uint2* ranges_enc, const uint32_t* n_dev) {
    switch (bits) {
        case 8: (void)radix_pass<8, 16>(ki, vi, ko, vo, n, shift, hist, s, ranges_enc, nullptr, n_dev); break;
        case 7: (void)radix_pass<7, 16>(ki, vi, ko, vo, n, shift, hist, s, ranges_enc, nullptr, n_dev); break;
        case 6: (void)radix_pass<6, 16>(ki, vi, ko, vo, n, shift, hist, s, ranges_enc, nullptr, n_dev); break;
        case 5: (void)radix_pass<5, 16>(ki, vi, ko, vo, n, shift, hist, s, ranges_enc, nullptr, n_dev); break;
        default: (void)radix_pass<4, 16>(ki, vi, ko, vo, n, shift, hist, s, ranges_enc, nullptr, n_dev); break;
    }
}

void launch_radix_sort_pairs(uint32_t* key_a, uint32_t* val_a, uint32_t* key_b, uint32_t* val_b, size_t n, int nbits,
                             uint32_t* hist, bool result_in_a, uint2* ranges_enc, hipStream_t s, const uint32_t* n_dev) {
    const int passes = (nbits + RADIX_BITS - 1) / RADIX_BITS;
    if (n == 0 || passes == 0) return;
    bool in_a = (passes % 2 == 0) ? result_in_a : !result_in_a;
    if (n <= (size_t)SMALL_SORT_MAX && (ranges_enc ? small_sort_usable<true>() : small_sort_usable<false>())) {
        const uint32_t* ki = in_a ? key_a : key_b;
        const uint32_t* vi = in_a ? val_a : val_b;
        uint32_t* ko = result_in_a ? key_a : key_b;
        uint32_t* vo = result_in_a ? val_a : val_b;
        const TotalsJob none = {nullptr, 0, nullptr, nullptr};
        if (ranges_enc)
            hipLaunchKernelGGL(small_sort_kernel<true>, dim3(1), dim3(SMALL_SORT_THREADS), sizeof(SmallSortLds), s, ki, vi, ko, vo,
                               (uint32_t)n, passes, none, ranges_enc, n_dev, OffsetSumsJob{nullptr, nullptr, nullptr});
        else
            hipLaunchKernelGGL(small_sort_kernel<false>, dim3(1), dim3(SMALL_SORT_THREADS), sizeof(SmallSortLds), s, ki, vi, ko, vo,
                               (uint32_t)n, passes, none, (uint2*)nullptr, n_dev, OffsetSumsJob{nullptr, nullptr, nullptr});
        return;
    }
    const DigitSplit split = tile_digit_split(nbits);
    for (int p = 0; p < passes; p++) {
        uint32_t* ki = in_a ? key_a : key_b;
        uint32_t* vi = in_a ? val_a : val_b;
        uint32_t* ko = in_a ? key_b : key_a;
        uint32_t* vo = in_a ? val_b : val_a;
        tile_radix_pass(split.width[p], ki, vi, ko, vo, n, split.shift[p], hist, s, p == passes - 1 ? ranges_enc : nullptr, n_dev);
        in_a = !in_a;
    }
}

hipError_t launch_depth_sort(const uint32_t* keys, uint32_t* key_a, uint32_t* val_a, uint32_t* key_b, uint32_t* val_b, size_t n,
                             uint32_t* hist, const TotalsJob* tj, hipStream_t s, const OffsetSumsJob* sums, bool* sums_done,
                             bool* counts_in_a) {
    if (sums_done) *sums_done = false;
    if (counts_in_a) *counts_in_a = false;
    if (n == 0) return hipSuccess;
    if (n <= (size_t)SMALL_SORT_MAX && small_sort_usable<false>()) {
        hipError_t rc = hipSuccess;
        const bool apart = tj && tj->partial && tj->ready;
        if (apart) {
            hipLaunchKernelGGL(totals_kernel, dim3(1), dim3(256), 0, s, *tj);
            rc = hipEventRecord(tj->ready, s);
        }
        hipLaunchKernelGGL(small_sort_kernel<false>, dim3(1), dim3(SMALL_SORT_THREADS), sizeof(SmallSortLds), s, keys, (const uint32_t*)nullptr,
                           key_a, val_a, (uint32_t)n, 4, (tj && tj->partial && !apart) ? *tj : TotalsJob{nullptr, 0, nullptr, nullptr},
                           (uint2*)nullptr, (const uint32_t*)nullptr, sums ? *sums : OffsetSumsJob{nullptr, nullptr, nullptr});
        if (sums && sums_done) *sums_done = true;
        return rc;
    }
    const uint32_t* const payload = (counts_in_a && sums) ? sums->tiles_touched : nullptr;
    if (n > 200000) {
        const hipError_t rc = radix_pass<RADIX_BITS, SORT_ITEMS>(keys, nullptr, key_b, val_b, n, 0, hist, s, nullptr, tj);
        (void)radix_pass<RADIX_BITS, SORT_ITEMS>(key_b, val_b, key_a, val_a, n, 8, hist, s);
        (void)radix_pass<RADIX_BITS, SORT_ITEMS>(key_a, val_a, key_b, val_b, n, 16, hist, s);
        (void)radix_pass<RADIX_BITS, SORT_ITEMS>(key_b, val_b, key_a, val_a, n, 24, hist, s, nullptr, nullptr, nullptr, payload);
        if (payload) *counts_in_a = true;
        return rc;
    }
    const hipError_t rc = radix_pass<DEPTH_RADIX_BITS, SORT_ITEMS>(keys, nullptr, key_a, val_a, n, 0, hist, s, nullptr, tj);
    (void)radix_pass<DEPTH_RADIX_BITS, SORT_ITEMS>(key_a, val_a, key_b, val_b, n, DEPTH_RADIX_BITS, hist, s);
    (void)radix_pass<DEPTH_RADIX_BITS, SORT_ITEMS>(key_b, val_b, key_a, val_a, n, 2 * DEPTH_RADIX_BITS, hist, s, nullptr, nullptr, nullptr,
                                                   payload);
    if (payload) *counts_in_a = true;
    return rc;
}


void launch_sort_prologue(const GeomState& g, size_t P, hipStream_t s) {
    const size_t nb = scan_blocks(P);
    if (nb == 0) return;
    hipLaunchKernelGGL(sort_prologue_kernel, dim3(nb), dim3(256), 0, s, g.depth_key, P, g.depth_hist, g.ref_partial,
                       (int)((P + 255) / 256), g.counters, g.lb_words, g.n_lb_words);
}

void launch_depth_sort_onesweep(const GeomState& g, size_t n, hipStream_t s) {
    if (n == 0) return;
    const uint32_t nb = (uint32_t)depth_sort_blocks(n);
    uint32_t* st = g.depth_status;
    const size_t st_stride = (size_t)nb * 256;
    uint2* const no_ranges = nullptr;
    hipLaunchKernelGGL((onesweep_pass_kernel<DEPTH_SORT_ITEMS, true, false>), dim3(nb), dim3(SORT_THREADS), 0, s, g.depth_key,
                       (const uint32_t*)nullptr, g.key_b, g.val_b, n, 0, g.depth_hist, st, g.tickets + 0, no_ranges);
    hipLaunchKernelGGL((onesweep_pass_kernel<DEPTH_SORT_ITEMS, true, false>), dim3(nb), dim3(SORT_THREADS), 0, s, g.key_b,
                       g.val_b, g.key_a, g.val_a, n, 8, g.depth_hist + 256, st + st_stride, g.tickets + 1, no_ranges);
    hipLaunchKernelGGL((onesweep_pass_kernel<DEPTH_SORT_ITEMS, true, false>), dim3(nb), dim3(SORT_THREADS), 0, s, g.key_a,
                       g.val_a, g.key_b, g.val_b, n, 16, g.depth_hist + 512, st + 2 * st_stride, g.tickets + 2, no_ranges);
    hipLaunchKernelGGL((onesweep_pass_kernel<DEPTH_SORT_ITEMS, false, false>), dim3(nb), dim3(SORT_THREADS), 0, s, g.key_b,
                       g.val_b, g.key_a, g.val_a, n, 24, g.depth_hist + 768, st + 3 * st_stride, g.tickets + 3, no_ranges);
}

void launch_tile_sort_onesweep(const GeomState& g, const BinState& b, size_t n, int passes, uint2* ranges, hipStream_t s) {
    if (n == 0) return;
    const uint32_t nb = (uint32_t)sort_blocks(n);
    const size_t st_stride = (size_t)nb * 256;
    if (passes == 1) {
        hipLaunchKernelGGL((onesweep_pass_kernel<SORT_ITEMS, true, true>), dim3(nb), dim3(SORT_THREADS), 0, s, b.tile_tmp,
                           b.id_tmp, b.tile_sorted, b.point_list, n, 0, g.tile_hist, b.tile_status, g.tickets + 5, ranges);
        return;
    }
    hipLaunchKernelGGL((onesweep_pass_kernel<SORT_ITEMS, true, false>), dim3(nb), dim3(SORT_THREADS), 0, s, b.tile_sorted,
                       b.point_list, b.tile_tmp, b.id_tmp, n, 0, g.tile_hist, b.tile_status, g.tickets + 5, (uint2*)nullptr);
    hipLaunchKernelGGL((onesweep_pass_kernel<SORT_ITEMS, true, true>), dim3(nb), dim3(SORT_THREADS), 0, s, b.tile_tmp,
                       b.id_tmp, b.tile_sorted, b.point_list, n, 8, g.tile_hist + 256, b.tile_status + st_stride,
                       g.tickets + 6, ranges);
}

void launch_radix_sort_keys_to_order(const uint32_t* keys, uint32_t* key_a, uint32_t* val_a, uint32_t* key_b, uint32_t* val_b,
                                     size_t n, int nbits, uint32_t* hist, hipStream_t s) {
    const int passes = (nbits + RADIX_BITS - 1) / RADIX_BITS;
    if (n == 0 || passes == 0) return;
    bool to_a = (passes % 2) == 1;
    const uint32_t* ki = keys;
    const uint32_t* vi = nullptr;
    for (int p = 0; p < passes; p++) {
        uint32_t* ko = to_a ? key_a : key_b;
        uint32_t* vo = to_a ? val_a : val_b;
        (void)radix_pass<RADIX_BITS, SORT_ITEMS>(ki, vi, ko, vo, n, p * RADIX_BITS, hist, s);
        ki = ko; vi = vo;
        to_a = !to_a;
    }
}

void launch_iota(uint32_t* dst, size_t n, hipStream_t s) {
    if (n) hipLaunchKernelGGL(iota_kernel, dim3((n + 255) / 256), dim3(256), 0, s, dst, n);
}

}
```

### feature-3dgs_amd/csrc/common.h

```cpp
#pragma once

#include <hip/hip_runtime.h>
#include <algorithm>
#include <stddef.h>
#include <stdint.h>

#include "../../include/f3dgs.h"

namespace f3dgs {

constexpr int TILE = 16;
constexpr int WAVE = 64;
constexpr size_t ALIGN = 256;

struct SplatRec {
    float4 q0, q1, q2;
};

constexpr int GREC = 12;

struct Carver {
    char* base;
    size_t off;
    explicit Carver(char* b) : base(b), off(0) {}
    template <typename T>
    T* take(size_t count) {
        off = (off + ALIGN - 1) & ~(ALIGN - 1);
        T* p = base ? reinterpret_cast<T*>(base + off) : nullptr;
        off += count * sizeof(T);
        return p;
    }
    size_t total() const { return (off + ALIGN - 1) & ~(ALIGN - 1); }
};

constexpr int RADIX_BITS = 8;
constexpr int RADIX_BINS = 1 << RADIX_BITS;
constexpr int DEPTH_RADIX_BITS = 11;
constexpr int DEPTH_RADIX_BINS = 1 << DEPTH_RADIX_BITS;
constexpr int SORT_THREADS = 256;
constexpr int SORT_ITEMS = 8;
constexpr int SORT_CHUNK = SORT_THREADS * SORT_ITEMS;
constexpr int SCAN_CHUNK = 256 * 16;
constexpr int SMALL_SORT_MAX = 16384;
constexpr int BIGQ_CAP = 1024;
constexpr int DEPTH_SORT_ITEMS = 8;

struct DigitSplit {
    int passes;
    int width[4], shift[4];
};
constexpr DigitSplit tile_digit_split(int bits) {
    DigitSplit s{};
    s.passes = (bits + RADIX_BITS - 1) / RADIX_BITS;
    const int w = s.passes ? (bits + s.passes - 1) / s.passes : 0;
    int at = 0;
    for (int p = 0; p < s.passes; p++) {
        s.width[p] = p + 1 < s.passes ? w : bits - at;
        s.shift[p] = at;
        at += s.width[p];
    }
    return s;
}
constexpr bool digit_split_ok(int bits) {
    const DigitSplit s = tile_digit_split(bits);
    if (s.passes != (bits + RADIX_BITS - 1) / RADIX_BITS) return false;
    int at = 0;
    for (int p = 0; p < s.passes; p++) {
        if (s.shift[p] != at || s.width[p] < 1 || s.width[p] > RADIX_BITS) return false;
        if (s.passes > 1 && s.width[p] < 4) return false;
        at += s.width[p];
    }
    return at == bits;
}
constexpr bool digit_splits_ok() {
    for (int bits = 1; bits <= 32; bits++)
        if (!digit_split_ok(bits)) return false;
    return true;
}
static_assert(digit_splits_ok(), "tile_digit_split: widths sum to the key's bits, each <= 8, contiguous shifts, ceil(bits / 8) passes");
static_assert(tile_digit_split(13).width[0] == 7 && tile_digit_split(13).width[1] == 6 && tile_digit_split(13).shift[1] == 7, "13 = 7 + 6");
static_assert(tile_digit_split(9).width[0] == 5 && tile_digit_split(9).width[1] == 4, "9 = 5 + 4");
static_assert(tile_digit_split(15).width[0] == 8 && tile_digit_split(15).width[1] == 7, "15 = 8 + 7");
static_assert(tile_digit_split(16).width[0] == 8 && tile_digit_split(16).width[1] == 8, "16 = 8 + 8");
static_assert(tile_digit_split(8).passes == 1 && tile_digit_split(8).width[0] == 8 && tile_digit_split(5).width[0] == 5, "one pass: the bits themselves");

inline size_t sort_blocks(size_t n) { return (n + SORT_CHUNK - 1) / SORT_CHUNK; }
inline size_t scan_blocks(size_t n) { return (n + SCAN_CHUNK - 1) / SCAN_CHUNK; }
inline size_t depth_sort_blocks(size_t n) { return (n + SORT_THREADS * DEPTH_SORT_ITEMS - 1) / (SORT_THREADS * DEPTH_SORT_ITEMS); }
inline size_t emit_blocks(size_t n) { return (n + 255) / 256; }

struct GeomState {
    SplatRec* rec;
    uint8_t* clamped;
    uint32_t* tiles_touched;
    uint32_t* depth_key;
    uint32_t* key_a;
    uint32_t* key_b;
    uint32_t* val_a;
    uint32_t* val_b;
    uint32_t* hist;
    uint32_t* scan_tmp;
    uint32_t* scan_sub;
    uint32_t* ref_partial;
    uint32_t* counters;
    uint32_t* depth_hist;
    uint32_t* big_ctl;
    uint2* big_items;
    uint32_t* lb_words;
    size_t n_lb_words;
    uint32_t* tickets;
    uint32_t* tile_hist;
    uint32_t* depth_status;
    uint32_t* emit_status;
    uint32_t* hist_copies;
    static GeomState carve(char* base, size_t P, size_t* bytes) {
        Carver c(base);
        GeomState g;
        g.rec = c.take<SplatRec>(P);
        g.clamped = c.take<uint8_t>(P);
        g.tiles_touched = c.take<uint32_t>(P);
        g.depth_key = c.take<uint32_t>(P);
        g.key_a = c.take<uint32_t>(P);
        g.key_b = c.take<uint32_t>(P);
        g.val_a = c.take<uint32_t>(P);
        g.val_b = c.take<uint32_t>(P);
        g.hist = c.take<uint32_t>(DEPTH_RADIX_BINS * sort_blocks(P) + DEPTH_RADIX_BINS);
        g.scan_tmp = c.take<uint32_t>(scan_blocks(P) + 8);
        g.scan_sub = c.take<uint32_t>(64 * scan_blocks(P));
        g.ref_partial = c.take<uint32_t>(3 * ((P + 255) / 256) + 3);
        g.counters = c.take<uint32_t>(16);
        g.depth_hist = c.take<uint32_t>(4 * 256);
        g.big_ctl = c.take<uint32_t>(4 + BIGQ_CAP);
        g.big_items = c.take<uint2>(BIGQ_CAP);
        g.n_lb_words = 8 + 2 * 256 + 4 * depth_sort_blocks(P) * 256 + emit_blocks(P) + 64 * 512;
        g.lb_words = c.take<uint32_t>(g.n_lb_words);
        g.tickets = g.lb_words;
        g.tile_hist = g.tickets + 8;
        g.depth_status = g.tile_hist + 2 * 256;
        g.emit_status = g.depth_status + 4 * depth_sort_blocks(P) * 256;
        g.hist_copies = g.emit_status + emit_blocks(P);
        if (bytes) *bytes = c.total();
        return g;
    }
};

struct BinState {
    uint32_t* point_list;
    uint32_t* tile_sorted;
    uint32_t* id_tmp;
    uint32_t* tile_tmp;
    uint32_t* hist;
    uint32_t* tile_status;
    uint2* ranges_enc;
    static const uint32_t* list_of(const char* base) { return reinterpret_cast<const uint32_t*>(base); }
    static BinState carve(char* base, size_t N, size_t* bytes, size_t tiles = 0) {
        Carver c(base);
        BinState b;
        b.point_list = c.take<uint32_t>(N);
        b.tile_sorted = c.take<uint32_t>(N);
        b.id_tmp = c.take<uint32_t>(N);
        b.tile_tmp = c.take<uint32_t>(N);
        b.hist = c.take<uint32_t>(RADIX_BINS * sort_blocks(N) + RADIX_BINS);
        b.tile_status = c.take<uint32_t>(2 * sort_blocks(N) * 256);
        b.ranges_enc = c.take<uint2>(tiles);
        if (bytes) *bytes = c.total();
        return b;
    }
};

struct ImageState {
    float* final_T;
    uint32_t* n_contrib;
    uint2* ranges;
    uint32_t* tile_len;
    uint32_t* tile_order;
    static ImageState carve(char* base, size_t HW, size_t tiles, size_t* bytes) {
        Carver c(base);
        ImageState s;
        s.final_T = c.take<float>(HW);
        s.n_contrib = c.take<uint32_t>(HW);
        s.ranges = c.take<uint2>(tiles);
        s.tile_len = c.take<uint32_t>(tiles);
        s.tile_order = c.take<uint32_t>(tiles);
        if (bytes) *bytes = c.total();
        return s;
    }
};

struct Options {
    int tile_cull;
    int feature_mfma;
    int profile;
    int bwd_half;
    int bwd_order;
    int bwd_m44;
    int bwd_split16;
    int bwd_bf16;
    int bwd_bf16_max_ratio;
    int bwd_wide8;
    int bwd_pl;
    int fwd_wide;
    int fwd_solo;
    int sort_onesweep;
    int sync_free;
    int instance_capacity;
    int knn_outward;
#ifdef F3DGS_DEV
    int dev;
#endif
};
Options& options();

struct ViewParams {
    const float* view;
    const float* proj;
    const float* campos;
    const float* bg;
    float tanx, tany, fx, fy;
    int W, H, gx, gy;
    int band0, band1;
    float scale_modifier;
    float max_axis_ratio;
};

void launch_mark_visible(int P, const float* means3D, const float* view_dev, uint8_t* present, hipStream_t s);
void launch_preprocess(int P, int D, int M, const float* means3D, const float* scales, const float* rotations,
                       const float* opacities, const float* shs, const float* cov3D_precomp,
                       const float* colors_precomp, const ViewParams& vp, int* radii, GeomState g, int cull, hipStream_t s);
void launch_preprocess_backward(int P, int D, int M, int C, const float* means3D, const int* radii, const float* shs,
                                const float* scales, const float* rotations, const float* cov3D_precomp,
                                const ViewParams& vp, const GeomState& g, const float* grec, float* dL_dmean2D,
                                float* dL_dconic, float* dL_dopacity, float* dL_dcolor, float* dL_dmean3D,
                                float* dL_dcov3D, float* dL_dsh, float* dL_dscale, float* dL_drot, float* dL_dz,
                                int row_begin, int row_end, hipStream_t s);
int preprocess_backward_row_align();

void launch_offset_sums(const uint32_t* in, const uint32_t* gather, size_t n, uint32_t* chunk_sums, uint32_t* sub,
                        hipStream_t s);
void launch_radix_sort_pairs(uint32_t* key_a, uint32_t* val_a, uint32_t* key_b, uint32_t* val_b, size_t n, int nbits,
                             uint32_t* hist, bool result_in_a, uint2* ranges_enc, hipStream_t s, const uint32_t* n_dev = nullptr);
void launch_emit_instances(int P, const GeomState& g, const uint32_t* order, const uint32_t* counts_in_order, int gx, int gy, int2 band, int cull,
                           uint32_t* inst_tile, uint32_t* inst_id, uint2* ranges_enc, uint32_t* tile_len, uint32_t cap,
                           const uint32_t* n_dev, uint32_t* overflow, hipStream_t s);
void launch_emit_scan(int P, const GeomState& g, const BinState& b, const uint32_t* order, int gx, int gy, int2 band, int cull,
                      uint32_t* inst_tile, uint32_t* inst_id, uint32_t N, uint2* ranges, hipStream_t s);
void launch_sort_prologue(const GeomState& g, size_t P, hipStream_t s);
void launch_depth_sort_onesweep(const GeomState& g, size_t n, hipStream_t s);
void launch_tile_sort_onesweep(const GeomState& g, const BinState& b, size_t n, int passes, uint2* ranges, hipStream_t s);
struct OffsetSumsJob {
    const uint32_t* tiles_touched;
    uint32_t* chunk_sums;
    uint32_t* sub;
};
struct TotalsJob {
    const uint32_t* partial;
    int n_partial;
    uint32_t* counters;
    uint32_t* host;
    hipEvent_t ready;
};
hipError_t launch_depth_sort(const uint32_t* keys, uint32_t* key_a, uint32_t* val_a, uint32_t* key_b, uint32_t* val_b, size_t n,
                             uint32_t* hist, const TotalsJob* tj, hipStream_t s, const OffsetSumsJob* sums = nullptr,
                             bool* sums_done = nullptr, bool* counts_in_a = nullptr);
void launch_iota(uint32_t* dst, size_t n, hipStream_t s);
void launch_radix_sort_keys_to_order(const uint32_t* keys, uint32_t* key_a, uint32_t* val_a, uint32_t* key_b, uint32_t* val_b,
                                     size_t n, int nbits, uint32_t* hist, hipStream_t s);

size_t feature_l1_scratch_bytes(int C, int Cout, int Hg, int Wg, bool decoder);
bool feature_l1_decoder_supported(int C);
const float* feature_l1_lowres_grad(char* scratch, int C, int Cout, int Hg, int Wg, bool decoder);
hipError_t launch_feature_l1(int C, int H, int W, int Cout, int Hg, int Wg, const float* feature_map, const float* weight,
                             const float* bias, const float* gt, float* loss, float* d_feature_map, float* d_weight,
                             float* d_bias, char* scratch, hipStream_t s);

size_t feature_decode_scratch_bytes(int C, int Hg, int Wg, bool decoder);
hipError_t launch_feature_decode(int C, int H, int W, int Cout, int Hg, int Wg, const float* feature_map, const float* weight,
                                 const float* bias, void* out, bool half, char* scratch, hipStream_t s);
void launch_feature_resize(int C, int H, int W, int Hg, int Wg, const float* feature_map, float* X, hipStream_t s);

size_t segment_scratch_bytes(int C, int Cout, int Hs, int Ws, int K, bool decoder);
hipError_t launch_segment(int C, int H, int W, int Cout, int Hs, int Ws, int K, const float* feature_map, const float* weight,
                          const float* bias, const float* text, bool round_half, bool text_normalized, int64_t* labels,
                          float* score, char* scratch, hipStream_t s);

size_t feature_pca_scratch_bytes(int C, size_t HW, int stride);
hipError_t launch_feature_pca_moments(int C, size_t HW, int stride, const float* feature_map, double* mean, double* cov,
                                      char* scratch, hipStream_t s);
hipError_t launch_feature_pca_project(int C, size_t HW, const float* feature_map, const float* mean, const float* components,
                                      const float* lo, const float* hi, float* out, hipStream_t s);

hipError_t launch_view_normals(int H, int W, const float* depth, const float* proj, const double* inv, float* out, bool chw, bool half,
                               hipStream_t s);
hipError_t launch_view_gradient(int Cn, int H, int W, const float* image, float* out, float* minmax, hipStream_t s);
hipError_t launch_view_curvature(int H, int W, const float* depth, const float* proj, const double* inv, float* out, float* minmax,
                                 hipStream_t s);
hipError_t launch_view_minmax(size_t n, const float* field, float* minmax, hipStream_t s);
hipError_t launch_view_palette(size_t HW, const float* field, const float* minmax, const float* lut, int L, int mode, float* out_float,
                               unsigned char* out_u8, hipStream_t s);
hipError_t launch_view_bytes(size_t HW, const float* image, unsigned char* out, hipStream_t s);

int report_error(int code, const char* msg);
int report_errorf(int code, const char* fmt, ...) __attribute__((format(printf, 2, 3)));

inline bool aligned16(const void* p) { return (reinterpret_cast<uintptr_t>(p) & 15) == 0; }

void launch_adam_step(size_t n, float* p, const float* g, float* m, float* v, double lr, double b1, double b2, double eps,
                      int step, const uint8_t* row_mask, size_t width, hipStream_t s);

void launch_adam_step_multi(int count, const f3dgs_adam_tensor* tensors, double b1, double b2, double eps, const uint8_t* row_mask,
                            size_t rows, hipStream_t s);

using DensifyTensor = f3dgs_densify_tensor;
constexpr int DENSIFY_MAX_TENSORS = F3DGS_DENSIFY_MAX_TENSORS;
constexpr int DENSIFY_ZERO_NEW = F3DGS_DENSIFY_ZERO_NEW, DENSIFY_OVERRIDE_CHILD = F3DGS_DENSIFY_OVERRIDE_CHILD;
void launch_densify_gather(size_t n_out, const int32_t* src_row, const uint8_t* kind, const int32_t* override_row, int n_tensors,
                           const DensifyTensor* tensors, hipStream_t s);

constexpr int KNN_LEAF = 256;
struct KnnBox {
    float lo[3], hi[3];
};
size_t knn_scratch_bytes(size_t P);
void launch_knn_sort(int P, const float* points, char* scratch, float4** sorted, KnnBox** leaf_box, int* n_leaf, hipStream_t s);
void launch_knn_mean_dist2(int P, const float* points, float* out, char* scratch, hipStream_t s);
hipError_t launch_knn_neighbors(int P, int K, const float* points, int* idx, float* dist2, char* scratch, bool outward, hipStream_t s);
hipError_t launch_label_mode_filter(int P, int K, const int* labels, const float* weight, const int* idx, const float* dist2,
                                    float max_dist2, bool fill, int* labels_out, float* share_out, hipStream_t s);

void launch_render_forward(const ViewParams& vp, int C, const uint2* ranges_enc, uint2* ranges, const uint32_t* point_list,
                           const SplatRec* rec, const float* feat, float* final_T,
                           uint32_t* n_contrib, float* out_color, float* out_feat, float* out_depth, uint32_t* tile_len,
                           hipStream_t s);
struct LowresGrad {
    const float* gx = nullptr;
    const float* scale = nullptr;
    int Hg = 0, Wg = 0;
};
int launch_render_backward(const ViewParams& vp, int C, const uint2* ranges, const uint32_t* point_list,
                           const SplatRec* rec, const float* final_T, const uint32_t* n_contrib,
                           const float* dL_dpix, const float* dL_dfeat, const float* dL_ddepth, float* grec,
                           float* dL_dfeature, const uint32_t* tile_len, uint32_t* tile_order, const LowresGrad* lowres,
                           int contraction, const uint32_t* gate, hipStream_t s);
struct WalkArgs {
    const uint2* ranges;
    const uint32_t* point_list;
    const SplatRec* rec;
    const uint32_t* n_contrib;
    int W, H, gx, gy;
    uint32_t band_b0, band_tb;
};
hipError_t launch_contributions(const WalkArgs& walk, int K, const float* masks, float* acc, float* wmax, float* alpha,
                                float* median_depth, int* ids, float* id_weight, hipStream_t s);
hipError_t launch_label_votes(const WalkArgs& walk, const void* labels, int format, int L, float* acc, hipStream_t s);
size_t instance_scratch_bytes(int M, int L);
hipError_t launch_instance_associate(int P, int M, int L, const float* acc_view, const float* acc, double iou_thresh, double min_weight,
                                     int* count, int* dropped, int* mapping, int* best_label, double* best_iou, float* table,
                                     char* scratch, hipStream_t s);
hipError_t launch_instance_merge(int P, int M, int L, float* acc_view, bool clear_view, const int* mapping, float* acc, hipStream_t s);
struct BwdArgs;
void launch_render_backward_pl(BwdArgs a, int C, hipStream_t s);
void launch_tile_order(const uint32_t* tile_len, size_t tiles, uint32_t* order, uint32_t band_b0, uint32_t band_tb, hipStream_t s);

#if defined(__HIPCC__)
__device__ __forceinline__ float wave_sum(float v) {
#pragma unroll
    for (int d = 32; d >= 1; d >>= 1) v += __shfl_xor(v, d, 64);
    return v;
}
__device__ __forceinline__ double wave_sum(double v) {
#pragma unroll
    for (int d = 32; d >= 1; d >>= 1) v += __shfl_xor(v, d, 64);
    return v;
}
template <typename T>
__device__ __forceinline__ T block_scan(T v, T* s_w, T& total) {
    const int lane = threadIdx.x & 63, wave = threadIdx.x >> 6;
    T inc = v;
    for (int d = 1; d < 64; d <<= 1) {
        const T o = __shfl_up(inc, d);
        if (lane >= d) inc += o;
    }
    __syncthreads();
    if (lane == 63) s_w[wave] = inc;
    __syncthreads();
    T before = 0;
    total = 0;
    for (int w = 0; w < 4; w++) {
        if (w < wave) before += s_w[w];
        total += s_w[w];
    }
    return before + inc - v;
}
__device__ __forceinline__ uint32_t xcd_remap(uint32_t b, uint32_t n) {
    constexpr uint32_t X = 8;
    const uint32_t q = n / X, r = n % X;
    const uint32_t xcd = b % X, k = b / X;
    const uint32_t start = xcd < r ? xcd * (q + 1) : r * (q + 1) + (xcd - r) * q;
    return start + k;
}
__host__ __device__ __forceinline__ uint32_t band_perm(uint32_t v, uint32_t T, uint32_t b0, uint32_t tb) {
    if (tb == 0) return v;
    constexpr uint32_t X = 8;
    const uint32_t q = T / X, r = T % X;
    const uint32_t x = v < r * (q + 1) ? v / (q + 1) : r + (v - r * (q + 1)) / q;
    const uint32_t f = x < r ? x * (q + 1) : r * (q + 1) + (x - r) * q;
    const uint32_t k = v - f;
    const uint32_t qb = tb / X, rb = tb % X;
    const uint32_t bf = x < rb ? x * (qb + 1) : rb * (qb + 1) + (x - rb) * qb;
    const uint32_t nb = x < rb ? qb + 1 : qb;
    if (k < nb) return b0 + bf + k;
    const uint32_t j = (f - bf) + (k - nb);
    return j < b0 ? j : j + tb;
}
#endif
inline void clamp_band(int begin, int end, int gy, int* band0, int* band1) {
    *band0 = std::min(std::max(begin, 0), gy);
// ... 12 lines not shown
```

### feature-3dgs_amd/csrc/preprocess.hip

```cpp

#include "common.h"
#include "lookback.h"

namespace f3dgs {

namespace {

struct M3 {
    float v[3][3];
};
__device__ __forceinline__ M3 mul3(const M3& A, const M3& B) {
    M3 R;
#pragma unroll
    for (int r = 0; r < 3; r++)
#pragma unroll
        for (int c = 0; c < 3; c++) R.v[r][c] = A.v[r][0] * B.v[0][c] + A.v[r][1] * B.v[1][c] + A.v[r][2] * B.v[2][c];
    return R;
}
__device__ __forceinline__ M3 tr3(const M3& A) {
    M3 R;
#pragma unroll
    for (int r = 0; r < 3; r++)
#pragma unroll
        for (int c = 0; c < 3; c++) R.v[r][c] = A.v[c][r];
// ... 188 lines not shown

constexpr int PF_ROW = 25;
template <int M3C>
__global__ void __launch_bounds__(256)
preprocess_kernel(int P, int D, int M, const float* __restrict__ means3D, const float* __restrict__ scales,
                  const float* __restrict__ rotations, const float* __restrict__ opacities,
                  const float* __restrict__ shs, const float* __restrict__ cov3D_precomp,
                  const float* __restrict__ colors_precomp, ViewParams vp, int* __restrict__ radii,
                  SplatRec* __restrict__ rec, uint8_t* __restrict__ clamped, uint32_t* __restrict__ tiles_touched,
                  uint32_t* __restrict__ depth_key, int cull, uint32_t* __restrict__ ref_partial,
                  uint32_t* __restrict__ depth_hist, uint32_t* __restrict__ big_ctl) {
    extern __shared__ __attribute__((aligned(16))) float sh_tile[];
    const int i = blockIdx.x * 256 + threadIdx.x;
    const int lane = threadIdx.x & 63, w = threadIdx.x >> 6;
    static_assert(BIGQ_CAP == 4 * 256, "slot states zeroed by workgroups 0..3 of this kernel, 256 words each");
    if (blockIdx.x < 4) {
        depth_hist[blockIdx.x * 256 + threadIdx.x] = 0;
        big_ctl[4 + blockIdx.x * 256 + threadIdx.x] = 0;
        if (blockIdx.x == 0 && threadIdx.x < 4) big_ctl[threadIdx.x] = 0;
    }
    int out_radius = 0;
    uint32_t out_tiles = 0, out_key = 0xFFFFFFFFu, bbox_tiles = 0;
    const size_t si = (size_t)(i < P ? i : 0);
    const V3 p = {means3D[3 * si], means3D[3 * si + 1], means3D[3 * si + 2]};
    const float opacity = opacities[si];
    const bool have_sr = !cov3D_precomp;
    const float* sp = have_sr ? scales + 3 * si : means3D + 3 * si;
    const float4* rp = have_sr ? reinterpret_cast<const float4*>(rotations) + si : reinterpret_cast<const float4*>(rec + si);
    const V3 sc_in = {sp[0], sp[1], sp[2]};
    const float4 q_in = *rp;
    bool alive = false;
    float px = 0.f, py = 0.f, ca = 0.f, cb = 0.f, cc = 0.f, rad = 0.f, depth = 0.f;
    bool long_axis = false;
    int x0 = 0, y0 = 0, x1 = 0, y1 = 0;
    if (i < P) do {
        const V3 pv = xform3(vp.view, p);
        if (pv.z <= 0.2f) break;
        const float* pm = vp.proj;
        const float hx = pm[0] * p.x + pm[4] * p.y + pm[8] * p.z + pm[12];
        const float hy = pm[1] * p.x + pm[5] * p.y + pm[9] * p.z + pm[13];
        const float hw = pm[3] * p.x + pm[7] * p.y + pm[11] * p.z + pm[15];
        const float pw = 1.0f / (hw + 0.0000001f);
        const float projx = hx * pw, projy = hy * pw;
        float cov6[6];
        if (cov3D_precomp) {
#pragma unroll
            for (int k = 0; k < 6; k++) cov6[k] = cov3D_precomp[6 * (size_t)i + k];
        } else {
            cov3d_from_scale_rot(sc_in, vp.scale_modifier, q_in, cov6);
        }
        const Ewa e = ewa_setup(p, vp, cov6);
        float a, b, c;
        ewa_cov(e, a, b, c);
        const float det = a * c - b * b;
        if (det == 0.0f) break;
        const float det_inv = 1.f / det;
        ca = c * det_inv; cb = -b * det_inv; cc = a * det_inv;
        const float mid = 0.5f * (a + c);
        const float root = sqrtf(fmaxf(0.1f, mid * mid - det));
        const float l1 = mid + root, l2 = mid - root;
        rad = ceilf(3.f * sqrtf(fmaxf(l1, l2)));
        px = ndc_to_pix(projx, vp.W); py = ndc_to_pix(projy, vp.H);
        tile_rect(px, py, (int)rad, vp.gx, make_int2(vp.band0, vp.band1), x0, y0, x1, y1);
        if ((x1 - x0) * (y1 - y0) == 0) break;
        depth = pv.z;
        alive = true;
        const float mr = vp.max_axis_ratio, lmax = fmaxf(l1, l2);
        long_axis = !(lmax * lmax <= (mr * mr) * det);
        if (have_sr) {
            const float s0 = fabsf(sc_in.x), s1 = fabsf(sc_in.y), s2 = fabsf(sc_in.z);
            long_axis = long_axis || !(fmaxf(s0, fmaxf(s1, s2)) <= mr * fminf(s0, fminf(s1, s2))) || fminf(s0, fminf(s1, s2)) == 0.f;
        }
    } while (false);

    float* const tile = sh_tile + w * (64 * PF_ROW);
    V3 col_part = {0.f, 0.f, 0.f};
    ShDir sdir = {0.f, 0.f, 0.f};
    if constexpr (M3C != 0) {
        static_assert(M3C == 48, "two halves of eight coefficients");
        const unsigned long long amask = __ballot(alive);
        const int wave_first = blockIdx.x * 256 + 64 * w;
        if (amask != 0ull) {
            constexpr int NH = 6;
            const float4* src = reinterpret_cast<const float4*>(shs + (size_t)wave_first * M3C);
            float4 q[2][NH];
#pragma unroll
            for (int h = 0; h < 2; h++)
#pragma unroll
                for (int k = 0; k < NH; k++) {
                    const int f = lane + 64 * k;
                    const int r = f / NH, c4 = f % NH;
                    const bool on = (amask >> r) & 1ull;
                    q[h][k] = src[on ? r * (M3C / 4) + h * NH + c4 : 0];
                }
            if (alive) sdir = sh_dir(p, vp.campos);
#pragma unroll
            for (int h = 0; h < 2; h++) {
#pragma unroll
                for (int k = 0; k < NH; k++) {
                    const int f = lane + 64 * k;
                    const int r = f / NH, c4 = f % NH;
                    if ((amask >> r) & 1ull) {
                        float* d = tile + r * PF_ROW + 4 * c4;
                        d[0] = q[h][k].x; d[1] = q[h][k].y; d[2] = q[h][k].z; d[3] = q[h][k].w;
                    }
                }
                __builtin_amdgcn_s_waitcnt(0xc07f);
                __builtin_amdgcn_wave_barrier();
                if (h == 0) {
                    if (alive && !colors_precomp) col_part = sh_first(D, sdir, tile + lane * PF_ROW);
                    __builtin_amdgcn_s_waitcnt(0xc07f);
                    __builtin_amdgcn_wave_barrier();
                }
            }
        }
    }

    if (alive) {
        V3 col;
        uint8_t cl = 0;
        if (colors_precomp) {
            col = {colors_precomp[3 * (size_t)i], colors_precomp[3 * (size_t)i + 1], colors_precomp[3 * (size_t)i + 2]};
        } else if constexpr (M3C != 0) {
            col = sh_second(D, sdir, col_part, tile + lane * PF_ROW, cl);
        } else {
            col = sh_to_rgb(D, p, vp.campos, shs + 3 * (size_t)M * i, cl);
        }
        SplatRec r;
        r.q0 = make_float4(px, py, ca, cb);
        r.q1 = make_float4(cc, opacity, col.x, col.y);
        r.q2 = make_float4(col.z, depth, __int_as_float((int)rad), 0.f);
        rec[i] = r;
        clamped[i] = cl;
        out_radius = (int)rad;
        bbox_tiles = (uint32_t)((y1 - y0) * (x1 - x0));
        if (cull) {
            const CullParams ck = make_cull(px, py, ca, cb, cc, opacity);
            const float cdet_inv = __builtin_amdgcn_rcpf(ca * cc - cb * cb);
            for (int ty = y0; ty < y1; ty++) {
                int xa, xb;
                if (row_span(ck, cdet_inv, ty, x0, x1, xa, xb)) out_tiles += (uint32_t)(xb - xa + 1);
            }
        } else {
            out_tiles = bbox_tiles;
        }
        out_key = __float_as_uint(depth);
    }
    if (i < P) {
        if (radii) radii[i] = out_radius;
        tiles_touched[i] = out_tiles;
        depth_key[i] = out_key;
        if (out_radius == 0) clamped[i] = 0;
    }
    __shared__ uint32_t wsum[3][4];
    uint32_t v = bbox_tiles, u = out_tiles;
    const uint32_t ar = __ballot(alive && long_axis) != 0ull ? 1u : 0u;
#pragma unroll
    for (int d = 32; d >= 1; d >>= 1) {
        v += (uint32_t)__shfl_xor((int)v, d, 64);
        u += (uint32_t)__shfl_xor((int)u, d, 64);
    }
    if ((threadIdx.x & 63) == 0) { wsum[0][threadIdx.x >> 6] = v; wsum[1][threadIdx.x >> 6] = u; wsum[2][threadIdx.x >> 6] = ar; }
    __syncthreads();
    if (threadIdx.x == 0) {
        const int nbp = (P + 255) / 256;
        if ((int)blockIdx.x < nbp) {
            ref_partial[blockIdx.x] = wsum[0][0] + wsum[0][1] + wsum[0][2] + wsum[0][3];
            ref_partial[nbp + blockIdx.x] = wsum[1][0] + wsum[1][1] + wsum[1][2] + wsum[1][3];
            ref_partial[2 * nbp + blockIdx.x] = max(max(wsum[2][0], wsum[2][1]), max(wsum[2][2], wsum[2][3]));
        }
    }
}

__device__ __forceinline__ void emit_big_splat(uint32_t gb, uint32_t o, const SplatRec* __restrict__ rec, int gx, int gy, int2 band, int cull,
                                               uint32_t* __restrict__ inst_tile, uint32_t* __restrict__ inst_id, int lane) {
    const float4 b0 = rec[gb].q0, b1 = rec[gb].q1;
    const int bradius = __float_as_int(rec[gb].q2.z);
    int bx0, by0, bx1, by1;
    tile_rect(b0.x, b0.y, bradius, gx, band, bx0, by0, bx1, by1);
    const CullParams bk = make_cull(b0.x, b0.y, b0.z, b0.w, b1.x, b1.y);
    const float bdet_inv = __builtin_amdgcn_rcpf(b0.z * b1.x - b0.w * b0.w);
    for (int yb = by0; yb < by1; yb += 64) {
        const int yl = yb + lane;
        int xa = bx0, n = 0;
        if (yl < by1) {
            int xb_ = bx1 - 1;
            if (!cull || row_span(bk, bdet_inv, yl, bx0, bx1, xa, xb_)) n = xb_ - xa + 1;
        }
        const uint32_t inc_r = wave_incl_scan((uint32_t)n, lane);
        const uint32_t roff = inc_r - (uint32_t)n;
        const uint32_t btot = (uint32_t)__shfl((int)inc_r, 63, 64);
        const int rows = min(64, by1 - yb);
        for (int r = 0; r < rows; r++) {
            const int nr = __builtin_amdgcn_readlane(n, r);
            if (nr == 0) continue;
            const int xar = __builtin_amdgcn_readlane(xa, r);
            const uint32_t ro = o + (uint32_t)__builtin_amdgcn_readlane((int)roff, r);
            const uint32_t t0 = (uint32_t)((yb + r) * gx + xar);
            for (int k = lane; k < nr; k += 64) {
                inst_tile[ro + k] = t0 + (uint32_t)k;
                inst_id[ro + k] = gb;
            }
        }
        o += btot;
    }
}

__device__ __forceinline__ uint32_t big_load(const uint32_t* p) { return __hip_atomic_load(p, __ATOMIC_RELAXED, __HIP_MEMORY_SCOPE_AGENT); }
__device__ __forceinline__ bool emit_big_claim(uint32_t* big_ctl, uint32_t slot, int lane) {
    uint32_t was = 0;
    if (lane == 0) was = atomicCAS(&big_ctl[4 + slot], 1u, 2u);
    return (uint32_t)__builtin_amdgcn_readfirstlane((int)was) == 1u;
}
__device__ __forceinline__ void emit_big_steal(uint32_t* big_ctl, const uint2* big_items, const SplatRec* __restrict__ rec, int gx, int gy, int2 band,
                                               int cull, uint32_t* __restrict__ inst_tile, uint32_t* __restrict__ inst_id, int lane) {
    for (;;) {
        const uint32_t handed = min(big_load(&big_ctl[0]), (uint32_t)BIGQ_CAP);
        if (big_load(&big_ctl[1]) >= handed) return;
        uint32_t i = 0;
        if (lane == 0) i = atomicAdd(&big_ctl[1], 1u);
        i = (uint32_t)__builtin_amdgcn_readfirstlane((int)i);
        if (i >= handed) return;
        if (emit_big_claim(big_ctl, i, lane)) {
            __threadfence();
            const uint32_t gb = big_load(&big_items[i].x), o = big_load(&big_items[i].y);
            emit_big_splat(gb, o, rec, gx, gy, band, cull, inst_tile, inst_id, lane);
        }
    }
}

constexpr int EMIT_CAP = 1024;
constexpr int EMIT_BIG = 512;
__global__ void __launch_bounds__(256)
emit_instances_kernel(int P, const uint32_t* __restrict__ order, const uint32_t* __restrict__ chunk_sums,
                      const uint32_t* __restrict__ sub, const uint32_t* __restrict__ tiles_touched,
                      const uint32_t* __restrict__ counts_in_order,
                      const SplatRec* __restrict__ rec, int gx, int gy, int2 band, int cull, uint32_t* __restrict__ inst_tile,
                      uint32_t* __restrict__ inst_id, uint2* __restrict__ ranges_enc, uint32_t* __restrict__ tile_len,
                      uint32_t* __restrict__ big_ctl, uint2* __restrict__ big_items, uint32_t cap, uint32_t* __restrict__ cap_word,
                      const uint32_t* __restrict__ n_dev, uint32_t* __restrict__ overflow) {
    __shared__ uint32_t s_tile[4][EMIT_CAP];
    __shared__ uint32_t s_id[4][EMIT_CAP];
    if (blockIdx.x == 0 && threadIdx.x == 0) *cap_word = cap;
    const bool no_room = n_dev && *n_dev > cap;
    if (no_room && overflow && blockIdx.x == 0 && threadIdx.x == 0)
        __hip_atomic_store(overflow, 1u, __ATOMIC_RELAXED, __HIP_MEMORY_SCOPE_SYSTEM);
    for (uint32_t t = blockIdx.x * 256 + threadIdx.x; t < (uint32_t)(gx * gy); t += gridDim.x * 256) {
        ranges_enc[t] = make_uint2(0xFFFFFFFFu, 0xFFFFFFFFu);
        tile_len[t] = 0u;
    }
    const int i = blockIdx.x * 256 + threadIdx.x;
    const int lane = threadIdx.x & 63, w = threadIdx.x >> 6;
    const bool valid = i < P;
    const uint32_t g = valid ? order[i] : 0u;
    const uint32_t cnt = valid ? (counts_in_order ? counts_in_order[i] : tiles_touched[g]) : 0u;
    const uint32_t first = (uint32_t)(blockIdx.x * 256 + 64 * w);
    const uint32_t chunk = first / SCAN_CHUNK, run = (first % SCAN_CHUNK) / 64;
    uint32_t before = (uint32_t)lane < run ? sub[(size_t)chunk * 64 + lane] : 0u;
    for (uint32_t c = lane; c < chunk; c += 64) before += chunk_sums[c];
#pragma unroll
    for (int d = 32; d >= 1; d >>= 1) before += (uint32_t)__shfl_xor((int)before, d, 64);
    const uint32_t base = before;
    const uint32_t inc = wave_incl_scan(cnt, lane);
    const uint32_t off0 = base + inc - cnt;
    const uint32_t total = (uint32_t)__shfl((int)inc, 63, 64);
    if (no_room || base + total > cap || base + total < base) return;
    const unsigned long long bigm = __ballot(cnt > (uint32_t)EMIT_BIG);
    if (bigm != 0ull) {
        const bool isbig = cnt > (uint32_t)EMIT_BIG;
        uint32_t slot0 = 0;
        if (lane == 0) slot0 = atomicAdd(&big_ctl[0], (uint32_t)__popcll(bigm));
        slot0 = (uint32_t)__builtin_amdgcn_readfirstlane((int)slot0);
        const uint32_t myslot = isbig ? slot0 + (uint32_t)__popcll(bigm & ((1ull << lane) - 1ull)) : 0xFFFFFFFFu;
        const bool queued = isbig && myslot < (uint32_t)BIGQ_CAP;
        if (queued) big_items[myslot] = make_uint2(g, off0);
        __threadfence();
        if (queued) __hip_atomic_store(&big_ctl[4 + myslot], 1u, __ATOMIC_RELEASE, __HIP_MEMORY_SCOPE_AGENT);
        if (cnt != 0 && cnt <= (uint32_t)EMIT_BIG) {
            uint32_t off_d = off0;
            const float4 d0 = rec[g].q0, d1 = rec[g].q1;
            const int dradius = __float_as_int(rec[g].q2.z);
            int dx0, dy0, dx1, dy1;
            tile_rect(d0.x, d0.y, dradius, gx, band, dx0, dy0, dx1, dy1);
            const CullParams dk = make_cull(d0.x, d0.y, d0.z, d0.w, d1.x, d1.y);
            const float ddet_inv = __builtin_amdgcn_rcpf(d0.z * d1.x - d0.w * d0.w);
            for (int y = dy0; y < dy1; y++) {
                int xa = dx0, xb = dx1 - 1;
                if (cull && !row_span(dk, ddet_inv, y, dx0, dx1, xa, xb)) continue;
                for (int x = xa; x <= xb; x++) {
                    inst_tile[off_d] = (uint32_t)(y * gx + x);
                    inst_id[off_d] = g;
                    off_d++;
                }
            }
        }
        emit_big_steal(big_ctl, big_items, rec, gx, gy, band, cull, inst_tile, inst_id, lane);
        for (unsigned long long m = bigm; m != 0ull; m &= m - 1ull) {
            const int b = __builtin_ctzll(m);
            const uint32_t slot = (uint32_t)__builtin_amdgcn_readlane((int)myslot, b);
            if (slot >= (uint32_t)BIGQ_CAP || emit_big_claim(big_ctl, slot, lane))
                emit_big_splat((uint32_t)__builtin_amdgcn_readlane((int)g, b), (uint32_t)__builtin_amdgcn_readlane((int)off0, b), rec, gx, gy, band,
                               cull, inst_tile, inst_id, lane);
        }
        return;
    }
    uint32_t off = off0;
    const uint32_t my_end = off0 + cnt;
    float4 q0 = make_float4(0.f, 0.f, 0.f, 0.f), q1 = q0;
    int x0 = 0, y0 = 0, x1 = 0, y1 = 0;
    CullParams ck{};
    float cdet_inv = 0.f;
    if (cnt != 0) {
        q0 = rec[g].q0; q1 = rec[g].q1;
        const int radius = __float_as_int(rec[g].q2.z);
        tile_rect(q0.x, q0.y, radius, gx, band, x0, y0, x1, y1);
        ck = make_cull(q0.x, q0.y, q0.z, q0.w, q1.x, q1.y);
        cdet_inv = __builtin_amdgcn_rcpf(q0.z * q1.x - q0.w * q0.w);
    }
    if (total <= (uint32_t)EMIT_CAP) {
        if (cnt != 0) {
            for (int y = y0; y < y1; y++) {
                int xa = x0, xb = x1 - 1;
// ... 451 lines not shown
```

### include/f3dgs.h

```cpp
#ifndef F3DGS_H_INCLUDED
#define F3DGS_H_INCLUDED

#include <stddef.h>
#include <stdint.h>

#ifdef __cplusplus
extern "C" {
#endif

#define F3DGS_OK 0
#define F3DGS_ERR_INVALID_ARGUMENT (-1)
#define F3DGS_ERR_HIP (-2)
#define F3DGS_ERR_ALLOC (-3)
#define F3DGS_ERR_UNSUPPORTED (-4)

typedef char* (*f3dgs_resize_fn)(void* ctx, size_t nbytes);

int f3dgs_version(void);

const char* f3dgs_last_error(void);

int f3dgs_set_option(const char* name, int value);
int f3dgs_get_option(const char* name, int* value );

int f3dgs_last_backward_contraction(void);
const uint32_t* f3dgs_forward_counts(void);
void f3dgs_set_tile_band(int tile_row_begin, int tile_row_end);
int f3dgs_debug_band_order(int gx, int gy, int tile_row_begin, int tile_row_end, uint32_t* tiles_out );
const char* f3dgs_option_name(int index);

int f3dgs_mark_visible(
    int P,
    const float* means3D,
    const float* viewmatrix,
    const float* projmatrix,
    uint8_t* present,
    void* stream );

int f3dgs_forward(
    f3dgs_resize_fn geometry_resize, void* geometry_ctx,
    f3dgs_resize_fn binning_resize, void* binning_ctx,
    f3dgs_resize_fn image_resize, void* image_ctx,
    int P, int D, int M, int C,
    const float* background,
    int width, int height,
    const float* means3D,
    const float* shs,
    const float* colors_precomp,
    const float* semantic_feature,
    const float* opacities,
    const float* scales,
    float scale_modifier,
    const float* rotations,
    const float* cov3D_precomp,
    const float* viewmatrix,
    const float* projmatrix,
    const float* cam_pos,
    float tan_fovx, float tan_fovy,
    int prefiltered,
    float* out_color,
    float* out_feature_map,
    float* out_depth,
    int* radii,
    int debug,
    void* stream ,
    int* num_rendered );

size_t f3dgs_backward_scratch_bytes(int P, int C);

int f3dgs_backward(
    int P, int D, int M, int C, int R,
    const float* background,
    int width, int height,
    const float* means3D,
    const float* shs,
    const float* colors_precomp,
    const float* semantic_feature,
    const float* scales,
    float scale_modifier,
    const float* rotations,
    const float* cov3D_precomp,
    const float* viewmatrix,
    const float* projmatrix,
    const float* campos,
    float tan_fovx, float tan_fovy,
    const int* radii,
    const char* geom_buffer,
    const char* binning_buffer,
    const char* image_buffer,
    const float* dL_dpix,
    const float* dL_dfeaturepix,
    const float* dL_depths,
    float* dL_dmean2D,
    float* dL_dconic,
    float* dL_dopacity,
    float* dL_dcolor,
    float* dL_dsemantic_feature,
    float* dL_dmean3D,
    float* dL_dcov3D,
    float* dL_dsh,
    float* dL_dscale,
    float* dL_drot,
    float* dL_dz,
    void* scratch,
    int debug,
    void* stream );

size_t f3dgs_feature_l1_scratch_bytes(int C, int Cout, int Hg, int Wg, int has_decoder);
int f3dgs_feature_l1(int C, int H, int W, int Cout, int Hg, int Wg, const float* feature_map, const float* weight,
                     const float* bias, const float* gt, float* loss, float* d_feature_map, float* d_weight,
                     float* d_bias, void* scratch, void* stream );

const float* f3dgs_feature_l1_lowres_grad(int C, int Cout, int Hg, int Wg, int has_decoder, void* scratch);

int f3dgs_set_feature_grad_lowres(const float* gx, int Hg, int Wg, const float* scale);

#define F3DGS_IMAGE_LOSS_L1_DSSIM 0
#define F3DGS_IMAGE_LOSS_SSIM 1
#define F3DGS_IMAGE_LOSS_SSIM_PER_IMAGE 2
size_t f3dgs_image_loss_scratch_bytes(int N, int C, int H, int W, int want_grad);
int f3dgs_image_loss_forward(int N, int C, int H, int W, const float* image, const float* gt, float lambda_dssim, int want_grad,
                             float* loss, float* l1, float* ssim, float* ssim_per_image, void* scratch, void* stream);
int f3dgs_image_loss_backward(int N, int C, int H, int W, const float* image, const float* gt, float lambda_dssim, int mode,
                              const float* upstream, const void* scratch, float* d_image, void* stream);

#define F3DGS_IMAGE_F32 0
#define F3DGS_IMAGE_U8_PLANAR 1
#define F3DGS_IMAGE_U8_INTERLEAVED 2
#define F3DGS_METRICS_QUANTIZE_IMAGE 0x1
#define F3DGS_METRICS_QUANTIZE_GT 0x2
size_t f3dgs_image_metrics_scratch_bytes(int N, int C, int H, int W);
int f3dgs_image_metrics(int N, int C, int H, int W, const void* image, int image_format, const void* gt, int gt_format, int flags,
                        float* l1 , float* mse , float* psnr , float* ssim , void* scratch,
                        void* stream );

#define F3DGS_EDIT_SELECT 0
#define F3DGS_EDIT_DELETE 1
#define F3DGS_EDIT_TEXT_NORMALIZED 0x100
#define F3DGS_EDIT_FILL_UNSELECTED 0x200
#define F3DGS_EDIT_MAX_TEXTS 64
#define F3DGS_EDIT_MAX_TEXT_ELEMENTS 32768
int f3dgs_edit_select(int P, int C, int K, const float* features, float* normalized_out, const float* text,
                      uint64_t positive_mask, int first_positive, int variant, int has_threshold, float threshold,
                      float* mask_out, float* score_out, const float* opacity_in, float* opacity_out,
                      void* stream );

#define F3DGS_CONTRIB_MAX_MASKS 7
int f3dgs_contributions(int P, int R, int width, int height,
                        const char* geom_buffer, const char* binning_buffer, const char* image_buffer,
                        int K, const float* masks , float* acc , float* wmax ,
                        float* alpha, float* median_depth, int* ids, float* id_weight ,
                        void* stream );

#define F3DGS_LABEL_VOTES_MAX_LABELS 65536
int f3dgs_label_votes(int P, int R, int width, int height,
                      const char* geom_buffer, const char* binning_buffer, const char* image_buffer,
                      const void* labels , int labels_format , int L,
                      float* acc , void* stream );

#define F3DGS_INSTANCE_MAX_MASKS 1024
#define F3DGS_INSTANCE_MAX_INSTANCES 4096
size_t f3dgs_instance_scratch_bytes(int M, int L);
int f3dgs_instance_associate(int P, int M, int L, const float* acc_view , const float* acc ,
                             double iou_thresh, double min_weight, int32_t* count, int32_t* dropped, int32_t* mapping ,
                             int32_t* best_label , double* best_iou , float* table ,
                             void* scratch, void* stream );
int f3dgs_instance_merge(int P, int M, int L, float* acc_view , int clear_view, const int32_t* mapping ,
                         float* acc , void* stream );

size_t f3dgs_feature_decode_scratch_bytes(int C, int Hg, int Wg, int has_decoder);
int f3dgs_feature_decode(int C, int H, int W, int Cout, int Hg, int Wg, const float* feature_map, const float* weight,
                         const float* bias, void* out, int out_is_half, void* scratch, void* stream);

#define F3DGS_SEGMENT_ROUND_HALF 0x1
#define F3DGS_SEGMENT_TEXT_NORMALIZED 0x2
#define F3DGS_SEGMENT_MAX_TEXTS 256
size_t f3dgs_segment_scratch_bytes(int C, int Cout, int Hs, int Ws, int K, int has_decoder);
int f3dgs_segment(int C, int H, int W, int Cout, int Hs, int Ws, int K, const float* feature_map, const float* weight,
                  const float* bias, const float* text , int flags, int64_t* labels ,
// ... 195 lines not shown
```

Before: 1713 Mpix/s.

## Sort Gaussians by depth with one bucket pass plus per-bucket LDS sorts

Replaces the multi-pass global LSD radix depth sort with a bucket sort for mid-sized P. Preprocessing now also reduces the per-block min and max depth keys. Keys are scattered into about 1024 linear depth buckets in a single global pass, then each bucket is radix-sorted inside LDS by its own workgroup, with oversized buckets handled by streaming passes. This cuts the number of full-array global passes over keys and values, in exchange for extra kernel complexity and load imbalance when the depth distribution is skewed.

After: 1739 Mpix/s (median of 6 runs). 1.5% higher.

```diff
diff --git a/feature-3dgs_amd/csrc/api.hip b/feature-3dgs_amd/csrc/api.hip
--- a/feature-3dgs_amd/csrc/api.hip
+++ b/feature-3dgs_amd/csrc/api.hip
@@ -271,6 +271,7 @@
     {"fwd_wide", "F3DGS_FWD_WIDE", &Options::fwd_wide, 1},
     {"fwd_solo", "F3DGS_FWD_SOLO", &Options::fwd_solo, 1},
     {"sort_onesweep", "F3DGS_SORT_ONESWEEP", &Options::sort_onesweep, 0},
+    {"depth_sort_buckets", "F3DGS_DEPTH_SORT_BUCKETS", &Options::depth_sort_buckets, -1},
     {"sync_free", "F3DGS_SYNC_FREE", &Options::sync_free, -1},
     {"instance_capacity", "F3DGS_INSTANCE_CAPACITY", &Options::instance_capacity, 0},
     {"knn_outward", "F3DGS_KNN_OUTWARD", &Options::knn_outward, 1},
@@ -319,6 +320,9 @@
 struct CountHint { bool known = false; uint32_t own = 0, ref = 0; };
 thread_local CountHint g_count_hint[64];
 thread_local const uint32_t* g_last_forward_words = nullptr;
+thread_local f3dgs::DepthSortInfo g_last_depth_sort = {F3DGS_DEPTH_SORT_NONE, 0u, 0u};
+thread_local bool g_depth_sort_known = false;
+thread_local uint32_t g_depth_sort_words[5];
 bool stream_is_capturing(hipStream_t s) {
     hipStreamCaptureStatus st = hipStreamCaptureStatusNone;
     if (hipStreamIsCapturing(s, &st) != hipSuccess) { (void)hipGetLastError(); return false; }
@@ -379,6 +383,18 @@
 int f3dgs_last_backward_contraction(void) { return g_last_bwd_bf16.load(); }
 
 const uint32_t* f3dgs_forward_counts(void) { return g_last_forward_words; }
+
+const uint32_t* f3dgs_depth_sort_info(void) {
+    if (!g_depth_sort_known) return nullptr;
+    const bool bk = g_last_depth_sort.path == F3DGS_DEPTH_SORT_BUCKETS && g_last_forward_words;
+    const volatile uint32_t* w = g_last_forward_words;
+    g_depth_sort_words[0] = (uint32_t)g_last_depth_sort.path;
+    g_depth_sort_words[1] = g_last_depth_sort.buckets;
+    g_depth_sort_words[2] = g_last_depth_sort.capacity;
+    g_depth_sort_words[3] = bk ? w[5] : 0u;
+    g_depth_sort_words[4] = bk ? w[6] : 0u;
+    return g_depth_sort_words;
+}
 
 int f3dgs_set_option(const char* name, int value) {
     if (!name) return fail(F3DGS_ERR_INVALID_ARGUMENT, "null option name");
@@ -544,8 +560,14 @@
     const OffsetSumsJob sums = {geom.tiles_touched, geom.scan_tmp, geom.scan_sub};
     bool sums_done = false;
     bool counts_in_a = false;
+    const int bk_opt = options().depth_sort_buckets;
+    const bool buckets = bk_opt > 0 || (bk_opt < 0 && (size_t)P > DEPTH_BUCKET_AUTO_ABOVE && (size_t)P <= DEPTH_BUCKET_AUTO_UPTO);
+    DepthSortInfo sort_info = {F3DGS_DEPTH_SORT_LOOKBACK, 0u, 0u};
     if (onesweep) launch_depth_sort_onesweep(geom, (size_t)P, s);
-    else HIP_TRY(launch_depth_sort(geom.depth_key, geom.key_a, geom.val_a, geom.key_b, geom.val_b, (size_t)P, geom.hist, &tj, s, &sums, &sums_done, &counts_in_a));
+    else HIP_TRY(launch_depth_sort(geom.depth_key, geom.key_a, geom.val_a, geom.key_b, geom.val_b, (size_t)P, geom.hist, &tj, s, &sums, &sums_done, &counts_in_a,
+                                   buckets, rb.dev + 5, &sort_info));
+    g_last_depth_sort = sort_info;
+    g_depth_sort_known = true;
     if ((rc = check_debug(debug, s, "depth sort"))) return rc;
     tm.mark("depth_sort");
     const uint32_t* order = geom.val_a;
diff --git a/feature-3dgs_amd/csrc/binding.cpp b/feature-3dgs_amd/csrc/binding.cpp
--- a/feature-3dgs_amd/csrc/binding.cpp
+++ b/feature-3dgs_amd/csrc/binding.cpp
@@ -1248,6 +1248,20 @@
         return py::make_tuple((long long)v[0], (long long)v[1], (long long)v[2], (long long)v[3], (long long)v[4]);
     }, "(entries of the instance lists, the reference's num_rendered, long-axis flag, entries provided for, sticky no-room word) of the "
        "calling thread's most recent forward call - final once that frame's work has completed; None before the first call");
+    m.def("depth_sort_info", []() -> py::object {
+        const uint32_t* w = f3dgs_depth_sort_info();
+        if (!w) return py::none();
+        py::dict d;
+        static const char* const names[] = {"none", "one_launch", "passes", "buckets", "lookback"};
+        d["path"] = w[0] < 5 ? names[w[0]] : "?";
+        d["buckets"] = (long long)w[1];
+        d["capacity"] = (long long)w[2];
+        d["largest"] = (long long)w[3];
+        d["oversized"] = (long long)w[4];
+        return d;
+    }, "how the calling thread's most recent forward call sorted its Gaussians by depth: path ('one_launch', 'passes', 'buckets', "
+       "'lookback', 'none'), and of the bucket path the bins in use, the in-LDS capacity of a bucket, the frame's largest bucket and "
+       "its buckets above the capacity (the last two final once the frame's work has completed); None before the first call");
     m.def("forward_counts_address", []() { return (uintptr_t)f3dgs_forward_counts(); },
           "host address of the five uint32 words of forward_counts() (0 before the first call): a captured step keeps it and reads the words after a replay");
     m.def("clear_forward_overflow", [](uintptr_t address) { if (address) reinterpret_cast<volatile uint32_t*>(address)[4] = 0u; },
diff --git a/feature-3dgs_amd/csrc/binning.hip b/feature-3dgs_amd/csrc/binning.hip
--- a/feature-3dgs_amd/csrc/binning.hip
+++ b/feature-3dgs_amd/csrc/binning.hip
@@ -62,11 +62,15 @@
     }
 }
 
-template <int BITS, int ITEMS>
+__device__ __forceinline__ uint32_t depth_bucket_of(uint32_t key, uint32_t kmin, uint32_t s, uint32_t culled_bin) {
+    return key == 0xFFFFFFFFu ? culled_bin : (key - kmin) >> s;
+}
+template <int BITS, int ITEMS, bool BUCKET = false>
 __global__ void __launch_bounds__(SORT_THREADS) radix_hist_kernel(const uint32_t* __restrict__ keys, size_t n,
                                                                   int shift, uint32_t nb,
                                                                   uint32_t* __restrict__ hist, TotalsJob tj,
-                                                                  const uint32_t* __restrict__ n_dev) {
+                                                                  const uint32_t* __restrict__ n_dev, uint32_t bucket_count,
+                                                                  uint32_t* __restrict__ ctl) {
     constexpr int BINS = 1 << BITS;
     constexpr int CHUNK = SORT_THREADS * ITEMS;
     __shared__ uint32_t h[BINS];
@@ -79,12 +83,34 @@
         key[k] = i < n ? keys[i] : 0u;
     }
     if (tj.partial && blockIdx.x == 0) run_totals_job<SORT_THREADS>(tj);
+    uint32_t kmin = 0, bshift = 0;
+    if constexpr (BUCKET) {
+        __shared__ uint32_t shk[2][SORT_THREADS / 64];
+        uint32_t lo = 0xFFFFFFFFu, hi = 0u;
+        for (int i = threadIdx.x; i < tj.n_partial; i += SORT_THREADS) {
+            lo = min(lo, tj.partial[3 * tj.n_partial + i]);
+            hi = max(hi, tj.partial[4 * tj.n_partial + i]);
+        }
+#pragma unroll
+        for (int d = 32; d >= 1; d >>= 1) {
+            lo = min(lo, (uint32_t)__shfl_xor((int)lo, d, 64));
+            hi = max(hi, (uint32_t)__shfl_xor((int)hi, d, 64));
+        }
+        if ((threadIdx.x & 63) == 0) { shk[0][threadIdx.x >> 6] = lo; shk[1][threadIdx.x >> 6] = hi; }
+        __syncthreads();
+        lo = min(min(shk[0][0], shk[0][1]), min(shk[0][2], shk[0][3]));
+        hi = max(max(shk[1][0], shk[1][1]), max(shk[1][2], shk[1][3]));
+        kmin = lo;
+        bshift = depth_bucket_shift(lo, hi, bucket_count);
+        if (blockIdx.x == 0 && threadIdx.x == 0) { ctl[0] = kmin; ctl[1] = bshift; }
+    }
     for (int d = threadIdx.x; d < BINS; d += SORT_THREADS) h[d] = 0;
     __syncthreads();
 #pragma unroll
     for (int k = 0; k < ITEMS; k++) {
         const size_t i = base + (size_t)k * SORT_THREADS + threadIdx.x;
-        if (i < n) atomicAdd(&h[(key[k] >> shift) & (BINS - 1)], 1u);
+        const uint32_t d = BUCKET ? depth_bucket_of(key[k], kmin, bshift, BINS - 1) : (key[k] >> shift) & (BINS - 1);
+        if (i < n) atomicAdd(&h[d], 1u);
     }
     __syncthreads();
     for (int d = threadIdx.x; d < BINS; d += SORT_THREADS) hist[(size_t)d * nb + blockIdx.x] = h[d];
@@ -135,15 +161,21 @@
     if (last) atomicMin(&ranges_enc[tile].y, 0xFFFFFFFFu - (pos + 1u));
 }
 
-template <int BITS, int ITEMS, bool REORDER, bool RANGES, bool COUNTS = false>
+template <int BITS, int ITEMS, bool REORDER, bool RANGES, bool COUNTS = false, bool BUCKET = false>
 __global__ void __launch_bounds__(SORT_THREADS)
 radix_scatter_kernel(const uint32_t* __restrict__ keys_in, const uint32_t* __restrict__ vals_in,
                      uint32_t* __restrict__ keys_out, uint32_t* __restrict__ vals_out, size_t n, int shift,
                      uint32_t nb, const uint32_t* __restrict__ hist, const uint32_t* __restrict__ totals,
                      uint2* __restrict__ ranges_enc, const uint32_t* __restrict__ n_dev,
-                     const uint32_t* __restrict__ payload) {
+                     const uint32_t* __restrict__ payload, const uint32_t* __restrict__ ctl, uint32_t* __restrict__ bucket_offs) {
     constexpr int BINS = 1 << BITS;
     constexpr int CHUNK = SORT_THREADS * ITEMS;
+    static_assert(!(BUCKET && (REORDER || RANGES || COUNTS)), "the bucket pass is a plain scatter of keys and ids");
+    const uint32_t bk_min = BUCKET ? ctl[0] : 0u, bk_shift = BUCKET ? ctl[1] : 0u;
+    auto digit_of = [&](uint32_t key) -> uint32_t {
+        if constexpr (BUCKET) return depth_bucket_of(key, bk_min, bk_shift, BINS - 1);
+        else return (key >> shift) & (BINS - 1);
+    };
     constexpr int BPT = BINS >= SORT_THREADS ? BINS / SORT_THREADS : 1;
     static_assert(BINS >= SORT_THREADS ? BINS % SORT_THREADS == 0 : true, "whole bins per thread");
     if (n_dev) {
@@ -178,7 +210,7 @@
     for (int k = 0; k < ITEMS; k++) {
         const size_t i = wbase + (size_t)k * 64 + lane;
         const bool valid = i < n;
-        const uint32_t d = (key[k] >> shift) & (BINS - 1);
+        const uint32_t d = digit_of(key[k]);
         const unsigned long long vm = __ballot(valid);
         uint32_t p_lo = (uint32_t)vm, p_hi = (uint32_t)(vm >> 32);
 #pragma unroll
@@ -222,6 +254,7 @@
             const uint32_t d = threadIdx.x * BPT + q;
             if (BINS < SORT_THREADS && d >= (uint32_t)BINS) break;
             const uint32_t g = digit_base + hist[(size_t)d * nb + blockIdx.x];
+            if (BUCKET && blockIdx.x == 0) bucket_offs[d] = digit_base;
             if (REORDER) { gbase[d] = g; lstart[d] = local_base; }
             uint32_t r2 = REORDER ? local_base : g;
 #pragma unroll
@@ -240,7 +273,7 @@
         for (int k = 0; k < ITEMS; k++) {
             const size_t i = wbase + (size_t)k * 64 + lane;
             if (i < n) {
-                const uint32_t d = (key[k] >> shift) & (BINS - 1);
+                const uint32_t d = digit_of(key[k]);
                 const uint32_t lp = cnt[w][d] + rank[k];
                 skey[lp] = key[k];
                 if constexpr (REORDER) sval[lp] = val[k];
@@ -288,7 +321,7 @@
         for (int k = 0; k < ITEMS; k++) {
             const size_t i = wbase + (size_t)k * 64 + lane;
             if (i < n) {
-                const uint32_t d = (key[k] >> shift) & (BINS - 1);
+                const uint32_t d = digit_of(key[k]);
                 const uint32_t pos = cnt[w][d] + rank[k];
                 if constexpr (COUNTS) {
                     keys_out[pos] = pay[k];
@@ -610,6 +643,306 @@
     return state[dev].load(std::memory_order_acquire) > 0;
 }
 
+struct BucketSortLds {
+    uint32_t key[DEPTH_BUCKET_CAP];
+    uint32_t val[DEPTH_BUCKET_CAP];
+    uint32_t cnt[DEPTH_BUCKET_THREADS / 64][256];
+    uint32_t wsum[4];
+    uint32_t red[2][DEPTH_BUCKET_THREADS / 64];
+};
+static_assert(2 * sizeof(BucketSortLds) <= 160 * 1024, "two workgroups per CU");
+static_assert(DEPTH_BUCKET_CAP >= 512, "the streaming passes keep their digit offsets in the key image");
+
+__device__ __forceinline__ uint32_t wave_digit_rank(uint32_t d, bool valid, volatile uint32_t* vcnt, unsigned long long lt_mask) {
+    const unsigned long long vm = __ballot(valid);
+    uint32_t p_lo = (uint32_t)vm, p_hi = (uint32_t)(vm >> 32);
+#pragma unroll
+    for (int b = 0; b < 8; b++) {
+        const uint32_t x = 0u - ((d >> b) & 1u);
+        const unsigned long long nm = ~__ballot(x != 0u);
+        p_lo &= (uint32_t)nm ^ x;
+        p_hi &= (uint32_t)(nm >> 32) ^ x;
+    }
+    const unsigned long long peers = ((unsigned long long)p_hi << 32) | p_lo;
+    const uint32_t before = __popcll(peers & lt_mask);
+    const uint32_t old = vcnt[d];
+    if (valid && before == 0) vcnt[d] = old + (uint32_t)__popcll(peers);
+    return old + before;
+}
+
+__device__ __forceinline__ uint32_t bucket_block_or(uint32_t v, uint32_t* red) {
+    constexpr int NW = DEPTH_BUCKET_THREADS / 64;
+#pragma unroll
+    for (int d = 32; d >= 1; d >>= 1) v |= (uint32_t)__shfl_xor((int)v, d, 64);
+    if ((threadIdx.x & 63) == 0) red[threadIdx.x >> 6] = v;
+    __syncthreads();
+    uint32_t r = 0;
+#pragma unroll
+    for (int k = 0; k < NW; k++) r |= red[k];
+    return r;
+}
+
+__device__ __forceinline__ void depth_bucket_stream_sort(BucketSortLds& L, uint32_t* key_b, uint32_t* val_b, uint32_t* key_a, uint32_t* val_a,
+                                                      uint32_t off, uint32_t n, uint32_t kmin, uint32_t low, uint32_t rel0,
+                                                      const uint32_t* __restrict__ payload) {
+    constexpr int THREADS = DEPTH_BUCKET_THREADS, ITEMS = 8, NW = THREADS / 64;
+    const int tid = threadIdx.x, lane = tid & 63, w = tid >> 6;
+    const unsigned long long lt_mask = (1ull << lane) - 1ull;
+    volatile uint32_t* vcnt = &L.cnt[w][0];
+    uint32_t diff = 0;
+    for (uint32_t j = tid; j < n; j += THREADS) diff |= ((key_b[off + j] - kmin) & low) ^ rel0;
+    diff = bucket_block_or(diff, L.red[0]);
+    int passes = (32 - __clz((int)diff) + 7) / 8;
+    if ((passes & 1) == 0) passes++;
+    uint32_t* const gbase = L.key;
+    uint32_t *sk = key_b, *sv = val_b, *dk = key_a, *dv = val_a;
+    for (int pass = 0; pass < passes; pass++) {
+        const int shift = 8 * pass;
+        const bool last = pass + 1 == passes;
+        auto digit_of = [&](uint32_t kk) -> uint32_t { return shift < 32 ? (((kk - kmin) & low) >> shift) & 255u : 0u; };
+        __syncthreads();
+        if (tid < 256) gbase[tid] = 0;
+        __syncthreads();
+        for (uint32_t j = tid; j < n; j += THREADS) atomicAdd(&gbase[digit_of(sk[off + j])], 1u);
+        __syncthreads();
+        {
+            const uint32_t tot = tid < 256 ? gbase[tid] : 0u;
+            uint32_t inc = tot;
+#pragma unroll
+            for (int d = 1; d < 64; d <<= 1) {
+                const uint32_t v = (uint32_t)__shfl_up((int)inc, d, 64);
+                if (lane >= d) inc += v;
+            }
+            if (tid < 256 && lane == 63) L.wsum[w] = inc;
+            __syncthreads();
+            if (tid < 256) {
+                uint32_t base = inc - tot;
+                for (int ww = 0; ww < w; ww++) base += L.wsum[ww];
+                gbase[tid] = base;
+            }
+        }
+        for (uint32_t c0 = 0; c0 < n; c0 += THREADS * ITEMS) {
+            for (int d = tid; d < NW * 256; d += THREADS) (&L.cnt[0][0])[d] = 0;
+            __syncthreads();
+            const uint32_t wbase = c0 + (uint32_t)(w * ITEMS * 64 + lane);
+            uint32_t key[ITEMS], val[ITEMS], rank[ITEMS];
+#pragma unroll
+            for (int k = 0; k < ITEMS; k++) {
+                const uint32_t i = wbase + (uint32_t)(k * 64);
+                const uint32_t ii = off + (i < n ? i : 0u);
+                key[k] = sk[ii];
+                val[k] = sv[ii];
+            }
+#pragma unroll
+            for (int k = 0; k < ITEMS; k++) {
+                const uint32_t i = wbase + (uint32_t)(k * 64);
+                rank[k] = wave_digit_rank(digit_of(key[k]), i < n, vcnt, lt_mask);
+            }
+            __syncthreads();
+            if (tid < 256) {
+                uint32_t base = gbase[tid];
+#pragma unroll
+                for (int ww = 0; ww < NW; ww++) {
+                    const uint32_t c = L.cnt[ww][tid];
+                    L.cnt[ww][tid] = base;
+                    base += c;
+                }
+                gbase[tid] = base;
+            }
+            __syncthreads();
+#pragma unroll
+            for (int k = 0; k < ITEMS; k++) {
+                const uint32_t i = wbase + (uint32_t)(k * 64);
+                if (i < n) {
+                    const uint32_t pos = off + L.cnt[w][digit_of(key[k])] + rank[k];
+                    dk[pos] = last ? payload[val[k]] : key[k];
+                    dv[pos] = val[k];
+                }
+            }
+            __syncthreads();
+        }
+        __threadfence();
+        __syncthreads();
+        __threadfence();
+        uint32_t* t = sk; sk = dk; dk = t;
+        t = sv; sv = dv; dv = t;
+    }
+}
+
+__global__ void __launch_bounds__(DEPTH_BUCKET_THREADS, 4)
+depth_bucket_sort_kernel(uint32_t* key_b, uint32_t* val_b, uint32_t* key_a, uint32_t* val_a, uint32_t bins,
+                         const uint32_t* __restrict__ totals, const uint32_t* __restrict__ offs, uint32_t* __restrict__ ctl,
+                         const uint32_t* __restrict__ payload, uint32_t* __restrict__ stats_host) {
+    extern __shared__ __attribute__((aligned(16))) char bucket_sort_smem[];
+    BucketSortLds& L = *reinterpret_cast<BucketSortLds*>(bucket_sort_smem);
+    constexpr int THREADS = DEPTH_BUCKET_THREADS, ITEMS = DEPTH_BUCKET_ITEMS, NW = THREADS / 64;
+    const int tid = threadIdx.x, lane = tid & 63, w = tid >> 6;
+    const uint32_t b = blockIdx.x;
+    if (b >= bins - 1u) {
+        const uint32_t off = offs[bins - 1u], n = totals[bins - 1u];
+        for (uint32_t j = (b - (bins - 1u)) * THREADS + tid; j < n; j += DEPTH_BUCKET_COPY_GROUPS * THREADS) {
+            const uint32_t id = val_b[off + j];
+            val_a[off + j] = id;
+            key_a[off + j] = payload[id];
+        }
+        if (b == bins - 1u) {
+            uint32_t mx = 0, over = 0;
+            for (uint32_t d = tid; d < bins - 1u; d += THREADS) {
+                const uint32_t t = totals[d];
+                mx = max(mx, t);
+                over += t > (uint32_t)DEPTH_BUCKET_CAP ? 1u : 0u;
+            }
+#pragma unroll
+            for (int d = 32; d >= 1; d >>= 1) {
+                mx = max(mx, (uint32_t)__shfl_xor((int)mx, d, 64));
+                over += (uint32_t)__shfl_xor((int)over, d, 64);
+            }
+            if (lane == 0) { L.red[0][w] = mx; L.red[1][w] = over; }
+            __syncthreads();
+            if (tid == 0) {
+                mx = 0; over = 0;
+                for (int k = 0; k < NW; k++) { mx = max(mx, L.red[0][k]); over += L.red[1][k]; }
+                ctl[2] = mx; ctl[3] = over;
+                if (stats_host) {
+                    __hip_atomic_store(&stats_host[0], mx, __ATOMIC_RELAXED, __HIP_MEMORY_SCOPE_SYSTEM);
+                    __hip_atomic_store(&stats_host[1], over, __ATOMIC_RELAXED, __HIP_MEMORY_SCOPE_SYSTEM);
+                    __threadfence_system();
+                }
+            }
+        }
+        return;
+    }
+    const uint32_t n = totals[b];
+    if (n == 0) return;
+    const uint32_t off = offs[b];
+    const uint32_t kmin = ctl[0], bshift = ctl[1];
+    const uint32_t low = (1u << bshift) - 1u;
+    const unsigned long long lt_mask = (1ull << lane) - 1ull;
+    const uint32_t rel0 = (key_b[off] - kmin) & low;
+    volatile uint32_t* vcnt = &L.cnt[w][0];
+
+    if (n <= (uint32_t)DEPTH_BUCKET_CAP) {
+        const int steps = (int)((n + THREADS - 1) / THREADS);
+        const uint32_t wbase = (uint32_t)(w * steps * 64 + lane);
+        uint32_t key[ITEMS], val[ITEMS], rank[ITEMS];
+        uint32_t diff = 0;
+#pragma unroll
+        for (int k = 0; k < ITEMS; k++) {
+            const uint32_t i = wbase + (uint32_t)(k * 64);
+            const bool mine = k < steps && i < n;
+            const uint32_t ii = mine ? off + i : off;
+            const uint32_t kk = key_b[ii];
+            val[k] = val_b[ii];
+            key[k] = mine ? (kk - kmin) & low : rel0;
+            diff |= key[k] ^ rel0;
+        }
+        diff = bucket_block_or(diff, L.red[0]);
+        const int passes = (32 - __clz((int)diff) + 7) / 8;
+        if (passes == 0) {
+#pragma unroll
+            for (int k = 0; k < ITEMS; k++) {
+                const uint32_t i = wbase + (uint32_t)(k * 64);
+                if (k < steps && i < n) {
+                    val_a[off + i] = val[k];
+                    key_a[off + i] = payload[val[k]];
+                }
+            }
+            return;
+        }
+        for (int pass = 0; pass < passes; pass++) {
+            const int shift = 8 * pass;
+            for (int d = tid; d < NW * 256; d += THREADS) (&L.cnt[0][0])[d] = 0;
+            __syncthreads();
+#pragma unroll
+            for (int k = 0; k < ITEMS; k++) {
+                if (k >= steps) break;
+                const uint32_t i = wbase + (uint32_t)(k * 64);
+                rank[k] = wave_digit_rank((key[k] >> shift) & 255u, i < n, vcnt, lt_mask);
+            }
+            __syncthreads();
+            {
+                uint32_t tot = 0;
+                if (tid < 256) {
+#pragma unroll
+                    for (int ww = 0; ww < NW; ww++) tot += L.cnt[ww][tid];
+                }
+                uint32_t inc = tot;
+#pragma unroll
+                for (int d = 1; d < 64; d <<= 1) {
+                    const uint32_t v = (uint32_t)__shfl_up((int)inc, d, 64);
+                    if (lane >= d) inc += v;
+                }
+                if (tid < 256 && lane == 63) L.wsum[w] = inc;
+                __syncthreads();
+                if (tid < 256) {
+                    uint32_t base = inc - tot;
+                    for (int ww = 0; ww < w; ww++) base += L.wsum[ww];
+#pragma unroll
+                    for (int ww = 0; ww < NW; ww++) {
+                        const uint32_t c = L.cnt[ww][tid];
+                        L.cnt[ww][tid] = base;
+                        base += c;
+                    }
+                }
+            }
+            __syncthreads();
+#pragma unroll
+            for (int k = 0; k < ITEMS; k++) {
+                const uint32_t i = wbase + (uint32_t)(k * 64);
+                if (k < steps && i < n) {
+                    const uint32_t pos = L.cnt[w][(key[k] >> shift) & 255u] + rank[k];
+                    L.key[pos] = key[k];
+                    L.val[pos] = val[k];
+                }
+            }
+            __syncthreads();
+            if (pass + 1 < passes) {
+#pragma unroll
+                for (int k = 0; k < ITEMS; k++) {
+                    const uint32_t i = wbase + (uint32_t)(k * 64);
+                    if (k < steps && i < n) { key[k] = L.key[i]; val[k] = L.val[i]; }
+                }
+            }
+        }
+        constexpr int HALF = ITEMS / 2;
+        for (int h = 0; h < 2; h++) {
+            if ((uint32_t)(h * HALF * THREADS) >= n) break;
+            uint32_t id[HALF], c[HALF];
+#pragma unroll
+            for (int k = 0; k < HALF; k++) {
+                const uint32_t j = (uint32_t)((h * HALF + k) * THREADS + tid);
+                id[k] = L.val[j < n ? j : 0u];
+                c[k] = payload[id[k]];
+            }
+#pragma unroll
+            for (int k = 0; k < HALF; k++) {
+                const uint32_t j = (uint32_t)((h * HALF + k) * THREADS + tid);
+                if (j < n) {
+                    val_a[off + j] = id[k];
+                    key_a[off + j] = c[k];
+                }
+            }
+        }
+        return;
+    }
+
+    depth_bucket_stream_sort(L, key_b, val_b, key_a, val_a, off, n, kmin, low, rel0, payload);
+}
+
+bool depth_bucket_sort_usable() {
+    constexpr int MAX_DEV = 64;
+    static std::atomic<int> state[MAX_DEV];
+    int dev = 0;
+    if (hipGetDevice(&dev) != hipSuccess || dev < 0 || dev >= MAX_DEV) return false;
+    if (state[dev].load(std::memory_order_acquire) == 0) {
+        const hipError_t e = hipFuncSetAttribute(reinterpret_cast<const void*>(&depth_bucket_sort_kernel),
+                                                 hipFuncAttributeMaxDynamicSharedMemorySize, (int)sizeof(BucketSortLds));
+        if (e != hipSuccess) (void)hipGetLastError();
+        state[dev].store(e == hipSuccess ? 1 : -1, std::memory_order_release);
+    }
+    return state[dev].load(std::memory_order_acquire) > 0;
+}
+
 template <int BITS, int ITEMS>
 static hipError_t radix_pass(const uint32_t* ki, const uint32_t* vi, uint32_t* ko, uint32_t* vo, size_t n, int shift,
                              uint32_t* hist, hipStream_t s, uint2* ranges_enc = nullptr, const TotalsJob* tj = nullptr,
@@ -620,23 +953,25 @@
     const uint32_t nb = (uint32_t)((n + SORT_THREADS * ITEMS - 1) / (SORT_THREADS * ITEMS));
     uint32_t* totals = hist + (size_t)BINS * nb;
     hipLaunchKernelGGL((radix_hist_kernel<BITS, ITEMS>), dim3(nb), dim3(SORT_THREADS), 0, s, ki, n, shift, nb, hist,
-                       tj ? *tj : TotalsJob{nullptr, 0, nullptr, nullptr}, n_dev);
+                       tj ? *tj : TotalsJob{nullptr, 0, nullptr, nullptr}, n_dev, 0u, (uint32_t*)nullptr);
     if (tj && tj->ready) rc = hipEventRecord(tj->ready, s);
     hipLaunchKernelGGL(radix_rowscan_kernel, dim3(BINS), dim3(256), 0, s, hist, nb, totals);
     const uint32_t* const no_payload = nullptr;
+    const uint32_t* const no_ctl = nullptr;
+    uint32_t* const no_offs = nullptr;
     if constexpr (ITEMS == SORT_ITEMS && (BITS == RADIX_BITS || BITS == DEPTH_RADIX_BITS)) {
         if (payload) {
             hipLaunchKernelGGL((radix_scatter_kernel<BITS, ITEMS, (BITS <= 8), false, true>), dim3(nb), dim3(SORT_THREADS), 0, s, ki,
-                               vi, ko, vo, n, shift, nb, hist, totals, (uint2*)nullptr, n_dev, payload);
+                               vi, ko, vo, n, shift, nb, hist, totals, (uint2*)nullptr, n_dev, payload, no_ctl, no_offs);
             return rc;
         }
     }
     if (ranges_enc && BITS <= 8)
         hipLaunchKernelGGL((radix_scatter_kernel<BITS, ITEMS, true, true>), dim3(nb), dim3(SORT_THREADS), 0, s, ki, vi, ko, vo, n,
-                           shift, nb, hist, totals, ranges_enc, n_dev, no_payload);
+                           shift, nb, hist, totals, ranges_enc, n_dev, no_payload, no_ctl, no_offs);
     else
         hipLaunchKernelGGL((radix_scatter_kernel<BITS, ITEMS, (BITS <= 8), false>), dim3(nb), dim3(SORT_THREADS), 0, s, ki, vi, ko,
-                           vo, n, shift, nb, hist, totals, (uint2*)nullptr, n_dev, no_payload);
+                           vo, n, shift, nb, hist, totals, (uint2*)nullptr, n_dev, no_payload, no_ctl, no_offs);
     return rc;
 }
 
@@ -683,9 +1018,10 @@
 
 hipError_t launch_depth_sort(const uint32_t* keys, uint32_t* key_a, uint32_t* val_a, uint32_t* key_b, uint32_t* val_b, size_t n,
                              uint32_t* hist, const TotalsJob* tj, hipStream_t s, const OffsetSumsJob* sums, bool* sums_done,
-                             bool* counts_in_a) {
+                             bool* counts_in_a, bool buckets, uint32_t* stats_host, DepthSortInfo* info) {
     if (sums_done) *sums_done = false;
     if (counts_in_a) *counts_in_a = false;
+    if (info) *info = DepthSortInfo{F3DGS_DEPTH_SORT_NONE, 0u, 0u};
     if (n == 0) return hipSuccess;
     if (n <= (size_t)SMALL_SORT_MAX && small_sort_usable<false>()) {
         hipError_t rc = hipSuccess;
@@ -698,9 +1034,44 @@
                            key_a, val_a, (uint32_t)n, 4, (tj && tj->partial && !apart) ? *tj : TotalsJob{nullptr, 0, nullptr, nullptr},
                            (uint2*)nullptr, (const uint32_t*)nullptr, sums ? *sums : OffsetSumsJob{nullptr, nullptr, nullptr});
         if (sums && sums_done) *sums_done = true;
+        if (info) info->path = F3DGS_DEPTH_SORT_ONE_LAUNCH;
         return rc;
     }
     const uint32_t* const payload = (counts_in_a && sums) ? sums->tiles_touched : nullptr;
+    if (buckets && payload && tj && tj->partial && n < (1ull << 31) && depth_bucket_sort_usable()) {
+        const uint32_t count = depth_bucket_count(n);
+        const uint32_t nb = (uint32_t)((n + SORT_THREADS * SORT_ITEMS - 1) / (SORT_THREADS * SORT_ITEMS));
+        const bool wide = depth_bucket_bits(n) == DEPTH_BUCKET_BITS_WIDE;
+        const uint32_t bins = 1u << depth_bucket_bits(n);
+        uint32_t* const totals = hist + (size_t)bins * nb;
+        uint32_t* const offs = totals + bins;
+        uint32_t* const ctl = offs + bins;
+        const uint32_t* const none = nullptr;
+        if (wide)
+            hipLaunchKernelGGL((radix_hist_kernel<DEPTH_BUCKET_BITS_WIDE, SORT_ITEMS, true>), dim3(nb), dim3(SORT_THREADS), 0, s, keys, n, 0,
+                               nb, hist, *tj, none, count, ctl);
+        else
+            hipLaunchKernelGGL((radix_hist_kernel<DEPTH_BUCKET_BITS, SORT_ITEMS, true>), dim3(nb), dim3(SORT_THREADS), 0, s, keys, n, 0,
+                               nb, hist, *tj, none, count, ctl);
+        hipError_t rc = hipSuccess;
+        if (tj->ready) rc = hipEventRecord(tj->ready, s);
+        hipLaunchKernelGGL(radix_rowscan_kernel, dim3(bins), dim3(256), 0, s, hist, nb, totals);
+        if (wide)
+            hipLaunchKernelGGL((radix_scatter_kernel<DEPTH_BUCKET_BITS_WIDE, SORT_ITEMS, false, false, false, true>), dim3(nb),
+                               dim3(SORT_THREADS), 0, s, keys, none, key_b, val_b, n, 0, nb, hist, totals, (uint2*)nullptr, none, none,
+                               (const uint32_t*)ctl, offs);
+        else
+            hipLaunchKernelGGL((radix_scatter_kernel<DEPTH_BUCKET_BITS, SORT_ITEMS, false, false, false, true>), dim3(nb),
+                               dim3(SORT_THREADS), 0, s, keys, none, key_b, val_b, n, 0, nb, hist, totals, (uint2*)nullptr, none, none,
+                               (const uint32_t*)ctl, offs);
+        hipLaunchKernelGGL(depth_bucket_sort_kernel, dim3(bins - 1u + DEPTH_BUCKET_COPY_GROUPS), dim3(DEPTH_BUCKET_THREADS),
+                           sizeof(BucketSortLds), s, key_b, val_b, key_a, val_a, bins, (const uint32_t*)totals, (const uint32_t*)offs, ctl,
+                           payload, stats_host);
+        *counts_in_a = true;
+        if (info) *info = DepthSortInfo{F3DGS_DEPTH_SORT_BUCKETS, count, (uint32_t)DEPTH_BUCKET_CAP};
+        return rc;
+    }
+    if (info) info->path = F3DGS_DEPTH_SORT_PASSES;
     if (n > 200000) {
         const hipError_t rc = radix_pass<RADIX_BITS, SORT_ITEMS>(keys, nullptr, key_b, val_b, n, 0, hist, s, nullptr, tj);
         (void)radix_pass<RADIX_BITS, SORT_ITEMS>(key_b, val_b, key_a, val_a, n, 8, hist, s);
diff --git a/feature-3dgs_amd/csrc/common.h b/feature-3dgs_amd/csrc/common.h
--- a/feature-3dgs_amd/csrc/common.h
+++ b/feature-3dgs_amd/csrc/common.h
@@ -83,6 +83,47 @@
 static_assert(tile_digit_split(15).width[0] == 8 && tile_digit_split(15).width[1] == 7, "15 = 8 + 7");
 static_assert(tile_digit_split(16).width[0] == 8 && tile_digit_split(16).width[1] == 8, "16 = 8 + 8");
 static_assert(tile_digit_split(8).passes == 1 && tile_digit_split(8).width[0] == 8 && tile_digit_split(5).width[0] == 5, "one pass: the bits themselves");
+
+constexpr int DEPTH_BUCKET_BITS = 10;
+constexpr int DEPTH_BUCKET_BITS_WIDE = 11;
+constexpr size_t DEPTH_BUCKET_WIDE_ABOVE = 1250000;
+constexpr int DEPTH_BUCKET_THREADS = 512;
+constexpr int DEPTH_BUCKET_ITEMS = 16;
+constexpr int DEPTH_BUCKET_CAP = 8064;
+constexpr int DEPTH_BUCKET_MEAN = 1024;
+constexpr int DEPTH_BUCKET_MIN_COUNT = 16;
+constexpr int DEPTH_BUCKET_COPY_GROUPS = 128;
+constexpr size_t DEPTH_BUCKET_AUTO_ABOVE = SMALL_SORT_MAX;
+constexpr size_t DEPTH_BUCKET_AUTO_UPTO = DEPTH_BUCKET_WIDE_ABOVE;
+static_assert(DEPTH_BUCKET_CAP <= DEPTH_BUCKET_THREADS * DEPTH_BUCKET_ITEMS && DEPTH_BUCKET_CAP % 64 == 0, "a bucket in LDS: whole waves, within the threads' items");
+static_assert(2 * (2 * 4 * DEPTH_BUCKET_CAP + 4 * 256 * (DEPTH_BUCKET_THREADS / 64) + 64) <= 160 * 1024, "two workgroups per CU");
+
+constexpr int depth_bucket_bits(size_t P) { return P > DEPTH_BUCKET_WIDE_ABOVE ? DEPTH_BUCKET_BITS_WIDE : DEPTH_BUCKET_BITS; }
+constexpr uint32_t depth_bucket_count(size_t P) {
+    const uint32_t most = 1u << depth_bucket_bits(P);
+    uint32_t c = DEPTH_BUCKET_MIN_COUNT;
+    while (c < most && (size_t)c * DEPTH_BUCKET_MEAN < P) c <<= 1;
+    return c;
+}
+#if defined(__HIPCC__)
+__host__ __device__
+#endif
+constexpr uint32_t depth_bucket_shift(uint32_t kmin, uint32_t kmax, uint32_t count) {
+    const uint32_t range = kmax > kmin ? kmax - kmin : 0u;
+    uint32_t s = 0;
+    while ((range >> s) > count - 2u) s++;
+    return s;
+}
+static_assert(depth_bucket_count(16385) == 32 && depth_bucket_count(16384) == 16 && depth_bucket_count(1) == 16, "mean bucket <= 1024, sixteen bins at least");
+static_assert(depth_bucket_count(1000000) == 1024 && depth_bucket_count(1250000) == 1024 && depth_bucket_count(1250001) == 2048 &&
+              depth_bucket_count(5000000) == 2048, "as many bins as the pass ranks bits, no more");
+static_assert(depth_bucket_shift(5, 5, 16) == 0 && depth_bucket_shift(0xFFFFFFFFu, 0u, 16) == 0, "one key or none: no shift, bucket 0");
+static_assert(depth_bucket_shift(0, 14, 16) == 0 && depth_bucket_shift(0, 15, 16) == 1, "the last bucket in use is count - 2");
+static_assert(depth_bucket_shift(0x40000000u, 0x41200000u, 1024) == 15, "z in 2 .. 10 over 1024 bins: 576 buckets of 2^15 keys");
+static_assert(depth_bucket_shift(0u, 0xFFFFFFFEu, 16) == 29 && (0xFFFFFFFEu >> 29) <= 14u, "the widest range stays below 32");
+
+constexpr int DEPTH_BUCKET_CTL_WORDS = 64;
+static_assert(DEPTH_BUCKET_BITS_WIDE <= DEPTH_RADIX_BITS, "GeomState::hist is sized for the widest depth pass");
 
 inline size_t sort_blocks(size_t n) { return (n + SORT_CHUNK - 1) / SORT_CHUNK; }
 inline size_t scan_blocks(size_t n) { return (n + SCAN_CHUNK - 1) / SCAN_CHUNK; }
@@ -124,10 +165,10 @@
         g.key_b = c.take<uint32_t>(P);
         g.val_a = c.take<uint32_t>(P);
         g.val_b = c.take<uint32_t>(P);
-        g.hist = c.take<uint32_t>(DEPTH_RADIX_BINS * sort_blocks(P) + DEPTH_RADIX_BINS);
+        g.hist = c.take<uint32_t>(DEPTH_RADIX_BINS * sort_blocks(P) + 2 * DEPTH_RADIX_BINS + DEPTH_BUCKET_CTL_WORDS);
         g.scan_tmp = c.take<uint32_t>(scan_blocks(P) + 8);
         g.scan_sub = c.take<uint32_t>(64 * scan_blocks(P));
-        g.ref_partial = c.take<uint32_t>(3 * ((P + 255) / 256) + 3);
+        g.ref_partial = c.take<uint32_t>(5 * ((P + 255) / 256) + 5);
         g.counters = c.take<uint32_t>(16);
         g.depth_hist = c.take<uint32_t>(4 * 256);
         g.big_ctl = c.take<uint32_t>(4 + BIGQ_CAP);
@@ -201,6 +242,7 @@
     int bwd_pl;
     int fwd_wide;
     int fwd_solo;
+    int depth_sort_buckets;
     int sort_onesweep;
     int sync_free;
     int instance_capacity;
@@ -259,9 +301,16 @@
     uint32_t* host;
     hipEvent_t ready;
 };
+struct DepthSortInfo {
+    int path;
+    uint32_t buckets;
+    uint32_t capacity;
+};
 hipError_t launch_depth_sort(const uint32_t* keys, uint32_t* key_a, uint32_t* val_a, uint32_t* key_b, uint32_t* val_b, size_t n,
                              uint32_t* hist, const TotalsJob* tj, hipStream_t s, const OffsetSumsJob* sums = nullptr,
-                             bool* sums_done = nullptr, bool* counts_in_a = nullptr);
+                             bool* sums_done = nullptr, bool* counts_in_a = nullptr, bool buckets = false,
+                             uint32_t* stats_host = nullptr, DepthSortInfo* info = nullptr);
+bool depth_bucket_sort_usable();
 void launch_iota(uint32_t* dst, size_t n, hipStream_t s);
 void launch_radix_sort_keys_to_order(const uint32_t* keys, uint32_t* key_a, uint32_t* val_a, uint32_t* key_b, uint32_t* val_b,
                                      size_t n, int nbits, uint32_t* hist, hipStream_t s);
diff --git a/feature-3dgs_amd/csrc/preprocess.hip b/feature-3dgs_amd/csrc/preprocess.hip
--- a/feature-3dgs_amd/csrc/preprocess.hip
+++ b/feature-3dgs_amd/csrc/preprocess.hip
@@ -364,15 +364,21 @@
         depth_key[i] = out_key;
         if (out_radius == 0) clamped[i] = 0;
     }
-    __shared__ uint32_t wsum[3][4];
+    __shared__ uint32_t wsum[5][4];
     uint32_t v = bbox_tiles, u = out_tiles;
+    uint32_t kmn = out_key, kmx = out_key == 0xFFFFFFFFu ? 0u : out_key;
     const uint32_t ar = __ballot(alive && long_axis) != 0ull ? 1u : 0u;
 #pragma unroll
     for (int d = 32; d >= 1; d >>= 1) {
         v += (uint32_t)__shfl_xor((int)v, d, 64);
         u += (uint32_t)__shfl_xor((int)u, d, 64);
-    }
-    if ((threadIdx.x & 63) == 0) { wsum[0][threadIdx.x >> 6] = v; wsum[1][threadIdx.x >> 6] = u; wsum[2][threadIdx.x >> 6] = ar; }
+        kmn = min(kmn, (uint32_t)__shfl_xor((int)kmn, d, 64));
+        kmx = max(kmx, (uint32_t)__shfl_xor((int)kmx, d, 64));
+    }
+    if ((threadIdx.x & 63) == 0) {
+        wsum[0][threadIdx.x >> 6] = v; wsum[1][threadIdx.x >> 6] = u; wsum[2][threadIdx.x >> 6] = ar;
+        wsum[3][threadIdx.x >> 6] = kmn; wsum[4][threadIdx.x >> 6] = kmx;
+    }
     __syncthreads();
     if (threadIdx.x == 0) {
         const int nbp = (P + 255) / 256;
@@ -380,6 +386,8 @@
             ref_partial[blockIdx.x] = wsum[0][0] + wsum[0][1] + wsum[0][2] + wsum[0][3];
             ref_partial[nbp + blockIdx.x] = wsum[1][0] + wsum[1][1] + wsum[1][2] + wsum[1][3];
             ref_partial[2 * nbp + blockIdx.x] = max(max(wsum[2][0], wsum[2][1]), max(wsum[2][2], wsum[2][3]));
+            ref_partial[3 * nbp + blockIdx.x] = min(min(wsum[3][0], wsum[3][1]), min(wsum[3][2], wsum[3][3]));
+            ref_partial[4 * nbp + blockIdx.x] = max(max(wsum[4][0], wsum[4][1]), max(wsum[4][2], wsum[4][3]));
         }
     }
 }
diff --git a/include/f3dgs.h b/include/f3dgs.h
--- a/include/f3dgs.h
+++ b/include/f3dgs.h
@@ -25,6 +25,12 @@
 
 int f3dgs_last_backward_contraction(void);
 const uint32_t* f3dgs_forward_counts(void);
+#define F3DGS_DEPTH_SORT_NONE 0
+#define F3DGS_DEPTH_SORT_ONE_LAUNCH 1
+#define F3DGS_DEPTH_SORT_PASSES 2
+#define F3DGS_DEPTH_SORT_BUCKETS 3
+#define F3DGS_DEPTH_SORT_LOOKBACK 4
+const uint32_t* f3dgs_depth_sort_info(void);
 void f3dgs_set_tile_band(int tile_row_begin, int tile_row_end);
 int f3dgs_debug_band_order(int gx, int gy, int tile_row_begin, int tile_row_end, uint32_t* tiles_out );
 const char* f3dgs_option_name(int index);
```
